# mbrea-c/bevy_firework

Measured on AMD Instinct MI355X. Metric: particles updated/sec (stress_test, 1M live), higher is better.
Workload: dtype f32; 1 GPU; configs[1]: 1 emitter x rate 1e6/s x lifetime 1 s per GPU (983 333 live), Point emission, linear 2-key scale/colour curves, dt=1/60, spawn + update + removal of the dead (order kept) every step; emitters_total=1, live_particles=983332, rccl_ranks=1, self_launched=False, update_mode=fused

## Files before the change

bevy_firework_amd/csrc/fw_engine.h:

```cpp
#pragma once
#include <hip/hip_runtime.h>

#include <algorithm>
#include <chrono>
#include <cmath>
#include <cstdio>
#include <cstdlib>
#include <cstring>
#include <string>
#include <deque>
#include <mutex>
#include <new>
#include <vector>

#include <sys/mman.h>
#include <immintrin.h>

#include "../../include/firework_hip.h"
#include "../../include/firework_hip_debug.h"
#include "fw_kernels.h"
#include "fw_math.h"
#include "fw_ages.h"
#include "fw_spin.h"
#include "fw_fuse2.h"
// ... 465 lines not shown
        if (n == cap) reserve_own(cap * 2);
        return p[n++];
    }
    void push_back(const FwOp &x) { push_slot() = x; }
    void append(const FwOp *b, const FwOp *e) {
        for (; b != e; ++b) push_back(*b);
    }
};

struct FwLevel {
    OpList g;
    std::vector<FwNestOp> n;
};

struct fw_ctx {
    std::vector<FwLevel> levels;
    OpList ops_scratch;
    std::vector<uint32_t> grow_scratch;
    HipBuf<char> d_stage;
    HipBuf<uint32_t> d_sort;
    bool seg_kind_changed = false;
    bool derive_ready_any = false;
    struct EmUndo {
        uint32_t spawner, entry;
        float last_emission, time_passed_in_cycle;
        bool enabled;
        uint64_t serial;
    };
    struct SpUndo {
        uint32_t spawner;
        uint64_t manual_queued_count;
    };
    std::vector<EmUndo> undo_em;
    std::vector<SpUndo> undo_sp;
    int device = 0;
    uint32_t seed = 0;
    HipStream stream, copy_stream;
    HipStream fifo_stream;
    HipEvent ev_side, ev_main;
    bool use_fifo_stream = true;
    bool side_dirty = false;
    bool fifo_last_side = false;
    bool main_reads_ring = false;
    std::string err;
    int update_mode = FW_MODE_FUSED;
    uint32_t spin_limit = 1u << 16;
    uint32_t dbg = 0;
    uint64_t recovered_rings = 0;

    std::vector<SpawnerHost, HugeAlloc<SpawnerHost>> spawners;
    std::vector<SegHost, HugeAlloc<SegHost>> segs;
    uint32_t n_types = 0, n_emits = 0, n_emit_slots = 0;
    std::vector<uint32_t> free_types, free_emits, free_emit_slots;
    size_t keys_end = 0;
    std::vector<std::pair<uint32_t, uint32_t>> free_keys;

    FwGlobals g{};
    struct {
        HipBuf<uint32_t> count, spawned, appended, rold;
        HipBuf<uint32_t> ndestroyed, range_ticket;
        HipBuf<uint32_t> tile_cnt, tile_off, err;
        HipBuf<unsigned long long> tile_status, dbg_ts, nest_status, nest_ticket, stats;
        HipBuf<float> tile_box;
    } gm;
    HipBuf<FwSeg> d_segs;
    HipBuf<FwType> d_types;
    HipBuf<FwTypeColl> d_type_coll;
    HipBuf<float> d_keys;
    HipBuf<FwEmit> d_emits;
    HipBuf<unsigned long long> d_emit_serial;
    HipBuf<uint32_t> d_nest_start;
    std::vector<uint32_t> nest_ticket_base;
    uint32_t max_seg = 0;
    size_t tiles_cap = 0;

    size_t param_bytes = 0;
    HipBuf<char> h_param[kParamRing];
    HipBuf<char> d_param[kParamRing];
    HipEvent ev_copied[kParamRing];
    Fence consumed[kParamRing];
    HipBuf<unsigned long long> h_done;
    unsigned long long *h_err = nullptr;
    std::string poison_msg;
    uint32_t n_poisoned = 0;
    uint64_t slot_frame[kParamRing] = {};

    HipBuf<unsigned long long> h_snap;
    bool snap_pending[kSnapRing] = {};
    bool snap_seen[kSnapRing] = {};
    uint32_t snap_epoch[kSnapRing] = {};
    std::vector<uint64_t> snap_cum[kSnapRing];

    HipBuf<uint32_t> d_tile_first;
    size_t tile_first_cap = 0;
    std::vector<uint32_t> tiles_dev;
    uint32_t total_tiles_dev = 0;
    HipBuf<uint32_t> h_tab[kTabRing];
    HipBuf<uint2> d_tile_keys;
    HipBuf<uint2> h_keys[kTabRing];
    HipBuf<uint4> d_tile_desc;
    HipBuf<uint4> h_desc[kTabRing];
    size_t tile_desc_cap = 0;
    Fence tab_fence[kTabRing];
    uint64_t tab_seq = 0, ring_seq = 0;
    uint32_t vt_rounds = 1;
    bool tab_force = false;

    uint32_t fc_sums_prev = 0;
    HipBuf<uint4> d_fce;
    HipBuf<unsigned long long> d_fc;
    size_t fc_len = 0;
    uint64_t fc_seq = 0;
    bool fc_dirty = false;
    bool fc_ok = false;
    uint32_t fc_dt_bits = 0;
    uint64_t fc_tab_seq = 0;
    bool use_forecast = true;
    bool use_tf = true;
    uint32_t tf_min_tiles = 768;
    HipBuf<uint4> d_fct;
    HipBuf<float2> d_fcl;
    size_t tf_cap = 0;
    uint32_t tf_armed = 0;
    float tf_prev_theta = 0.0f;
    uint64_t tf_frames = 0;
    bool use_static_new = true;
    bool use_stream = true;
    bool track_aabb = false;
    uint32_t boxes_epoch = 0;
    bool colors_dirty = false;
    bool use_fifo = true;
    bool fifo_nested = true;
    bool use_nospin = true;
    bool use_ageless = true;
    struct CohortTable {
        Staging<char, 1> h;
        HipBuf<char> d;
        uint64_t launches = 0;
    };
    CohortTable age_tab;
    bool use_spin_defer = true;
    uint32_t spin_defer_min = 384u * FW_TILE, spin_defer_after = 32u, spin_log_cap = 256u;
    CohortTable spin_tab;
    bool use_spinless = true;
    uint64_t spinless_launches = 0;
    bool use_whole_tiles = true;
    uint64_t whole_launches = 0, whole_tiles = 0;
    bool newborn_spin = false;
    uint64_t newborn_launches = 0;
    bool use_fuse2 = true;
    uint32_t fuse2_min = 384u * FW_TILE;
    uint32_t fuse_depth = FW_FUSE_MAX, fuse_deep_min = 768u * FW_TILE, fuse_wide_min = 768u * FW_TILE;
    uint32_t fuse_far_depth = FW_FUSE_FAR_DEFAULT, fuse_far_min = 768u * FW_TILE;
    FwWithheld withheld;
    uint64_t fused_launches = 0, fuse2_flushed = 0, fuse_frames = 0;
    bool use_axis = true;
    bool use_derived = true;
    bool derive_all = true;
    uint32_t fifo_small_tiles = 384;
    uint32_t fifo_min = 32768;
    FwPathCensus census;
    bool use_small = true;
    uint32_t small_max = 768;
    uint32_t wave_all_min = 896;
    bool wave_all_on = false;
    uint32_t wide_min = 768;
    bool wide_on = false;
    bool wide_mid_on = false;
    uint32_t wide_mid = 1400;
    uint32_t wide_max = 2048;
    uint32_t n_narrow = 0;
    uint32_t small_min = 352;
    bool small_last_side = false;
    bool small_on = false;
    bool host_fast = true;
    std::vector<uint32_t> big_list;
    bool big_dirty = true;
    std::vector<uint32_t> small_list;
    bool small_dirty = true;
    HipBuf<uint32_t> d_small, h_small;
    size_t small_cap = 0;
    Fence small_fence;
    std::vector<FwOp> fifo_ops;
    std::vector<std::pair<uint32_t, FwOp>> range_mat_ops;
    std::vector<std::pair<uint32_t, FwOp>> fifo_mat_ops;
    uint64_t tev_frames = 0;
    bool use_range = true;
    uint32_t range_min = 8192;
    uint32_t range_few = 192;
    uint32_t range_small_tiles = 384;
    bool range_small = false;
    uint32_t range_young_rounds = 4;
    uint32_t range_young_big = 0;
    std::vector<FwOp> range_ops;
    struct BirthAge {
        uint64_t frame;
        float age;
    };
    std::deque<BirthAge> birth_age;
    float range_life_max = 0.f;
    float range_age_keep = 0.f;
    HipBuf<FwRangeDesc> d_rdesc;
    HipBuf<FwRangeDesc> h_rdesc;
    size_t rdesc_cap = 0;
    uint32_t r_total = 0;
    bool r_force = true;
    Fence rtab_fence;
    HipBuf<unsigned long long> d_rstatus;
    HipBuf<char> h_rparam[kParamRing];
    bool param_bar = false;
    HipBuf<char> b_param[kParamRing];
    bool range_spread_new = true;
    uint64_t nt_bytes = 768ull << 20;
    uint64_t nt_wo_bytes = 280ull << 20, nt_wo_bytes_range = 64ull << 20;
    HipBuf<unsigned long long> d_rts;
    std::vector<uint32_t> range_scratch;
    size_t rparam_bytes = 0;
    uint64_t rslot_frame[kParamRing] = {};
    uint64_t rring_seq = 0;
    uint64_t r_uploads = 0;

    uint32_t nest_seq = 0;
    bool nest_fuse = true;
    uint64_t fused_nest_frames = 0, nest_pass_frames = 0;
    bool trace = false;
    bool host_prof = false;
    uint64_t host_prof_skip = 0;
    double prof_ns[10] = {};
    uint64_t prof_frames = 0;
    uint64_t frame = 0;
    double sim_time = 0.0;
    uint32_t parity = 0;
    unsigned long long stats_before_last = 0;
    bool stats_valid = false;

    bool timing = false;
    std::vector<HipEvent> tev;
    size_t tev_used = 0;
    uint64_t timing_particles_start = 0;
    double tev_overhead_ms = 0;

    unsigned long long *live_ring = nullptr;
    uint32_t live_ring_n = 0;
    uint64_t live_ring_frames = 0;

    HipBuf<FwCollider> d_colliders;
    uint32_t n_colliders = 0;
    Staging<FwCollider, 2> h_coll;
    struct MeshHost {
        bool alive = false;
        HipBuf<float4> nodes, tris;
        uint32_t n_nodes = 0, n_tris = 0;
        float center[3] = {0.0f, 0.0f, 0.0f}, radius = 0.0f;
        bool deformable = false;
        uint32_t n_vertices = 0;
        HipBuf<FwSlotIdx> slots;
        HipBuf<uint32_t> order, level_off;
        HipBuf<float> xyz;
        Staging<float, 2> h_xyz;
        std::vector<uint32_t> h_level_off;
        std::vector<uint8_t> referenced;
        float lo[3] = {0.0f, 0.0f, 0.0f}, hi[3] = {0.0f, 0.0f, 0.0f}, pad = 0.0f;
        HipBuf<FwMeshRecord> d_rec;
        HipBuf<FwVtxAcc> d_partials;
        HipBuf<uint8_t> d_referenced;
        HipBuf<FwMeshReport> h_report;
        bool dev_bounds = false;
        uint64_t sphere_stamp = 0;
    };
    static constexpr int kMeshDeviceAllocs = 4;
    std::vector<MeshHost> meshes;
    std::vector<fw_mesh> mesh_set;
    std::vector<fw_mesh_collider> mesh_insts;
    HipBuf<FwMeshInst> d_mesh_inst;
    Staging<FwMeshInst, 2> h_mesh_inst;
    HipBuf<float4> q_in_h, q_out_h, q_in_d, q_out_d;
    HipBuf<float4> q_out2_h, q_out2_d;
    HipBuf<float> d_aabb;
    HipBuf<float> h_aabb;
    struct {
        Staging<char, 2> h_tab;
        HipBuf<char> d_tab;
        HipBuf<float> d_part;
        HipBuf<float> h_out;
        std::vector<uint32_t> place_first;
        uint64_t launches = 0, last_chunks = 0;
    } boxes;
    struct {
        HipBuf<uint32_t> d_part;
        HipBuf<uint32_t> h_out;
        uint64_t launches = 0, last_chunks = 0;
    } volumes;
    HipBuf<unsigned long long> d_total;
    HipBuf<uint32_t> d_segids;

    uint64_t fail_alloc = 0, n_alloc = 0;

    fw_ctx() = default;
    fw_ctx(const fw_ctx &) = delete;
    fw_ctx &operator=(const fw_ctx &) = delete;
    ~fw_ctx();
};

namespace fwh {


// ... 255 lines not shown
```

bevy_firework_amd/csrc/fw_engine_api.cpp:

```cpp
#include "fw_engine.h"

thread_local std::string fwh::g_create_error;

static bool host_maps_writable(const void *p) {
    FILE *f = fopen("/proc/self/maps", "r");
    if (!f) return false;
    char line[512];
    bool ok = false;
    const unsigned long long a = (unsigned long long)(uintptr_t)p;
    while (fgets(line, sizeof line, f)) {
        unsigned long long lo = 0, hi = 0;
        char perms[8] = {0};
        if (sscanf(line, "%llx-%llx %7s", &lo, &hi, perms) == 3 && a >= lo && a < hi) {
            ok = perms[0] == 'r' && perms[1] == 'w';
            break;
        }
    }
    fclose(f);
    return ok;
}

static fw_status create_resources(fw_ctx *ctx, hipStream_t stream) {
    if (stream)
        ctx->stream.borrow(stream);
// ... 15 lines not shown
    return ensure_max_seg(ctx, 1024);
}

fw_ctx::~fw_ctx() {
    for (hipStream_t s : {(hipStream_t)stream, (hipStream_t)copy_stream, (hipStream_t)fifo_stream})
        if (s) (void)hipStreamSynchronize(s);
}

enum class Then { nothing, sync, join, counts };
enum class Ages { leave, ages, write };
struct SpawnerCall {
    SpawnerHost *sp = nullptr;
    std::vector<uint32_t> c;
    fw_status st = FW_OK;
};
template <typename ArgsOk>
static bool begin_call(fw_ctx *ctx, fw_spawner h, SpawnerCall &r, Then then, Ages ages, ArgsOk args_ok) {
    r.sp = get_spawner(ctx, h);
    if (!r.sp || !args_ok(*r.sp)) return r.st = FW_EINVAL, false;
    if (poll_device_error(ctx), r.sp->poisoned) return r.st = poisoned_status(ctx), false;
    hipSetDevice(ctx->device);
    if ((r.st = flush_withheld(ctx))) return false;
    for (size_t t = 0; ages != Ages::leave && t < r.sp->seg.size(); t++)
        if ((ages == Ages::write && (r.st = ensure_spin(ctx, r.sp->seg[t]))) || (r.st = ensure_ages(ctx, r.sp->seg[t]))) return false;
    r.st = then == Then::sync ? sync(ctx) : then == Then::join ? join_side(ctx) : then == Then::counts ? read_counts(ctx, r.c) : FW_OK;
    return !r.st || (then == Then::counts && r.st == FW_ECAPACITY);
}

static fw_status clear_poison_report(fw_ctx *ctx) {
    poll_device_error(ctx);
    ctx->h_err[0] = ctx->h_err[1] = 0ull;
    const uint32_t zero = 0;
    FW_HIP(ctx, hipMemcpy(ctx->g.err, &zero, sizeof zero, hipMemcpyHostToDevice));
    return FW_OK;
}

static void recount_poisoned(fw_ctx *ctx) {
    ctx->n_poisoned = 0;
    for (const SpawnerHost &x : ctx->spawners) ctx->n_poisoned += (x.alive && x.poisoned) ? 1u : 0u;
}

static fw_status check_handles(fw_ctx *ctx, uint32_t n, const fw_spawner *handles, const char *msg) {
    for (uint32_t i = 0; i < n; i++)
        if (!get_spawner(ctx, handles[i])) return fail(ctx, FW_EINVAL, msg);
    return FW_OK;
}

static int lplane_of(const SegHost &S, uint32_t emission_index) {
    int plane = -1;
    for (uint32_t k = 0; k < S.n_lplanes; k++)
        if (S.lplane_emission[k] == (int32_t)emission_index) plane = (int)k;
    return plane;
}

static fw_status read_stat_total(fw_ctx *ctx, uint64_t *total) {
    unsigned long long slots[FW_STAT_SLOTS];
    FW_HIP(ctx, hipMemcpy(slots, ctx->g.stats, sizeof slots, hipMemcpyDeviceToHost));
    *total = 0;
    for (unsigned long long v : slots) *total += v;
    return FW_OK;
}

extern "C" {


int fw_abi_version(void) { return FW_ABI_VERSION; }

const char *fw_last_error(const fw_ctx *ctx) { return ctx ? ctx->err.c_str() : g_create_error.c_str(); }

uint64_t fw_compute_emission_count(float t, float last, float dur, float start, float end, float per_cycle,
                                   float *next_last) {
    float nl = 0.f;
    const uint64_t n = fw_emission_count(t, last, dur, start, end, per_cycle, &nl);
    if (next_last) *next_last = nl;
    return n;
}

fw_status fw_ctx_create(int device, uint32_t seed, void *stream, fw_ctx **out) {
    if (!out) return FW_EINVAL;
    *out = nullptr;
    int ndev = 0;
    hipError_t e = hipGetDeviceCount(&ndev);
    if (e != hipSuccess || ndev <= 0) {
        g_create_error = std::string("no HIP device available (") + hipGetErrorString(e) +
                         "); this backend has no CPU fallback";
        return FW_ENODEV;
    }
    if (device < 0 || device >= ndev) {
        g_create_error = "device index out of range";
        return FW_EINVAL;
    }
    if ((e = hipSetDevice(device)) != hipSuccess) {
        g_create_error = std::string("hipSetDevice: ") + hipGetErrorString(e);
        return FW_ENODEV;
    }
    hipDeviceProp_t prop;
    if (hipGetDeviceProperties(&prop, device) == hipSuccess && strncmp(prop.gcnArchName, "gfx950", 6) != 0) {
        g_create_error = std::string("kernels are built for gfx950 only; device is ") + prop.gcnArchName;
        return FW_ENODEV;
    }
    fw_ctx *ctx = new fw_ctx();
    ctx->device = device;
    ctx->seed = seed;
    const char *knobs_on = getenv("FW_ENABLE_KNOBS");
    auto getenv = [&](const char *name) -> const char * { return (knobs_on && atoi(knobs_on) != 0) ? ::getenv(name) : nullptr; };
#ifdef FW_AB
    if (const char *m = getenv("FW_FAIL_ALLOC")) ctx->fail_alloc = strtoull(m, nullptr, 10);
#endif
    {
        int large_bar = 0;
        HipBuf<char> probe;
        if (hipDeviceGetAttribute(&large_bar, hipDeviceAttributeIsLargeBar, device) == hipSuccess && large_bar != 0 &&
            alloc_buf(ctx, probe, 4096, Mem::fine) == FW_OK) {
            hipPointerAttribute_t at{};
            ctx->param_bar = hipPointerGetAttributes(&at, probe) == hipSuccess && at.type == hipMemoryTypeDevice && host_maps_writable(probe);
        }
        (void)hipGetLastError();
        ctx->err.clear();
    }
    ctx->g.seed = seed;
    if (const char *m = getenv("FW_UPDATE_MODE")) ctx->update_mode = !strcmp(m, "split") ? FW_MODE_SPLIT : FW_MODE_FUSED;
    if (const char *m = getenv("FW_FORECAST")) ctx->use_forecast = atoi(m) != 0;
    if (const char *m = getenv("FW_TF")) ctx->use_tf = atoi(m) != 0;
    if (const char *m = getenv("FW_TF_MIN_TILES")) ctx->tf_min_tiles = (uint32_t)strtoul(m, nullptr, 10);
    if (const char *m = getenv("FW_STREAM")) ctx->use_stream = atoi(m) != 0;
    if (const char *m = getenv("FW_STATIC_NEW")) ctx->use_static_new = atoi(m) != 0;
    if (const char *m = getenv("FW_SPIN_LIMIT")) ctx->spin_limit = (uint32_t)strtoul(m, nullptr, 10);
    if (const char *m = getenv("FW_FIFO")) ctx->use_fifo = atoi(m) != 0;
    if (const char *m = getenv("FW_FIFO_MIN")) ctx->fifo_min = (uint32_t)strtoul(m, nullptr, 10);
    if (const char *m = getenv("FW_FIFO_SMALL")) ctx->fifo_small_tiles = (uint32_t)strtoul(m, nullptr, 10);
    if (const char *m = getenv("FW_FIFO_STREAM")) ctx->use_fifo_stream = atoi(m) != 0;
    if (const char *m = getenv("FW_RANGE")) ctx->use_range = atoi(m) != 0;
    if (const char *m = getenv("FW_RANGE_MIN")) ctx->range_min = (uint32_t)strtoul(m, nullptr, 10);
    if (const char *m = getenv("FW_RANGE_FEW")) ctx->range_few = (uint32_t)strtoul(m, nullptr, 10);
    if (const char *m = getenv("FW_RANGE_SMALL")) ctx->range_small_tiles = (uint32_t)strtoul(m, nullptr, 10);
    if (const char *m = getenv("FW_RANGE_YOUNG_BIG")) ctx->range_young_big = (uint32_t)strtoul(m, nullptr, 10);
    if (const char *m = getenv("FW_NOSPIN")) ctx->use_nospin = atoi(m) != 0;
    if (const char *m = getenv("FW_AXIS_SPIN")) ctx->use_axis = atoi(m) != 0;
    if (const char *m = getenv("FW_AGELESS")) ctx->use_ageless = atoi(m) != 0;
    if (const char *m = getenv("FW_SPIN_DEFER")) ctx->use_spin_defer = atoi(m) != 0;
    if (const char *m = getenv("FW_SPIN_DEFER_MIN")) ctx->spin_defer_min = (uint32_t)strtoul(m, nullptr, 10);
    if (const char *m = getenv("FW_SPIN_DEFER_AFTER")) ctx->spin_defer_after = (uint32_t)strtoul(m, nullptr, 10);
    if (const char *m = getenv("FW_SPIN_LOG")) ctx->spin_log_cap = (uint32_t)strtoul(m, nullptr, 10);
    if (const char *m = getenv("FW_SPINLESS")) ctx->use_spinless = atoi(m) != 0;
    if (const char *m = getenv("FW_WHOLE_TILES")) ctx->use_whole_tiles = atoi(m) != 0;
    if (const char *m = getenv("FW_NEWBORN_SPIN")) ctx->newborn_spin = atoi(m) != 0;
    if (const char *m = getenv("FW_FUSE2")) ctx->use_fuse2 = atoi(m) != 0;
    if (const char *m = getenv("FW_FUSE2_MIN")) ctx->fuse2_min = (uint32_t)strtoul(m, nullptr, 10);
    if (const char *m = getenv("FW_FUSE_DEPTH")) ctx->fuse_depth = (uint32_t)std::min(std::max(atoi(m), 2), (int)FW_FUSE_MAX);
    if (const char *m = getenv("FW_FUSE_DEEP_MIN")) ctx->fuse_deep_min = (uint32_t)strtoul(m, nullptr, 10);
    if (const char *m = getenv("FW_FUSE_WIDE_MIN")) ctx->fuse_wide_min = (uint32_t)strtoul(m, nullptr, 10);
    if (const char *m = getenv("FW_FUSE_FAR_DEPTH")) ctx->fuse_far_depth = (uint32_t)std::min(std::max(atoi(m), (int)FW_FUSE_MAX), (int)FW_FUSE_FAR);
    if (const char *m = getenv("FW_FUSE_FAR_MIN")) ctx->fuse_far_min = (uint32_t)strtoul(m, nullptr, 10);
    if (const char *m = getenv("FW_DERIVED")) ctx->use_derived = atoi(m) != 0, ctx->derive_all = atoi(m) >= 2;
    if (const char *m = getenv("FW_NEST_FUSE")) ctx->nest_fuse = atoi(m) != 0;
    if (const char *m = getenv("FW_SMALL")) ctx->use_small = atoi(m) != 0;
    if (const char *m = getenv("FW_SMALL_MAX")) ctx->small_max = (uint32_t)strtoul(m, nullptr, 10);
    if (const char *m = getenv("FW_SMALL_MIN")) ctx->small_min = (uint32_t)strtoul(m, nullptr, 10);
    if (const char *m = getenv("FW_WIDE_MAX")) ctx->wide_max = (uint32_t)strtoul(m, nullptr, 10);
    if (const char *m = getenv("FW_WIDE_MIN")) ctx->wide_min = (uint32_t)strtoul(m, nullptr, 10);
    if (const char *m = getenv("FW_WIDE_MID")) ctx->wide_mid = (uint32_t)strtoul(m, nullptr, 10);
    if (const char *m = getenv("FW_WAVE_ALL_MIN")) ctx->wave_all_min = (uint32_t)strtoul(m, nullptr, 10);
    if (const char *m = getenv("FW_HOST_FAST")) ctx->host_fast = atoi(m) != 0;
    if (const char *m = getenv("FW_PARAM_BAR")) ctx->param_bar = ctx->param_bar && atoi(m) != 0;
    if (const char *m = getenv("FW_NT_MB")) ctx->nt_bytes = (uint64_t)atoll(m) << 20;
    if (const char *m = getenv("FW_NT_WO_MB")) ctx->nt_wo_bytes = ctx->nt_wo_bytes_range = (uint64_t)atoll(m) << 20;
#ifdef FW_AB
    if (const char *m = getenv("FW_DEBUG")) ctx->dbg = (uint32_t)atoi(m);
    if (const char *m = getenv("FW_FIFO_NESTED")) ctx->fifo_nested = atoi(m) != 0;
    if (const char *m = getenv("FW_RANGE_SPREAD_NEW")) ctx->range_spread_new = atoi(m) != 0;
    if (const char *m = getenv("FW_AABB")) ctx->track_aabb = atoi(m) != 0;
    ctx->trace = getenv("FW_TRACE") != nullptr;
    if (const char *m = getenv("FW_HOST_PROF")) ctx->host_prof = atoi(m) != 0, ctx->host_prof_skip = atoi(m) > 1 ? (uint64_t)atoi(m) : 0;
#endif
    if (create_resources(ctx, (hipStream_t)stream) != FW_OK) {
        g_create_error = ctx->err;
        delete ctx;
        return FW_EHIP;
    }
    *out = ctx;
    return FW_OK;
}

fw_status fw_ctx_destroy(fw_ctx *ctx) {
    if (!ctx) return FW_EINVAL;
    hipSetDevice(ctx->device);
    drop_withheld(ctx);
    if (ctx->host_prof && ctx->prof_frames) {
        static const char *names[10] = {"windows+reset", "spawner loop", "tile table", "commit", "args", "op tables", "launch", "post", "", ""};
        fprintf(stderr, "[fw] host half of fw_step over %llu frames (ns per frame):", (unsigned long long)ctx->prof_frames);
        for (int i = 0; i < 8; i++) fprintf(stderr, "  %s %.0f", names[i], ctx->prof_ns[i] / (double)ctx->prof_frames);
        fprintf(stderr, "\n[fw] table uploads: general %llu, range %llu over %llu frames\n", (unsigned long long)ctx->tab_seq,
                (unsigned long long)ctx->r_uploads, (unsigned long long)ctx->frame);
        fprintf(stderr, "[fw] host records: SegHost %zu B, SpawnerHost %zu B (entry at %zu), EmissionHost %zu B, FwOp %zu B\n", sizeof(SegHost),
                sizeof(SpawnerHost), (size_t)((const char *)&ctx->spawners.data()->em.one_ - (const char *)ctx->spawners.data()),
                sizeof(EmissionHost), sizeof(FwOp));
    }
    delete ctx;
    return FW_OK;
}

void *fw_ctx_stream(const fw_ctx *ctx) { return ctx ? (void *)ctx->stream : nullptr; }

fw_status fw_ctx_synchronize(fw_ctx *ctx) {
    if (!ctx) return FW_EINVAL;
    fw_status st = sync(ctx);
    if (st) return st;
    return check_device_errors(ctx);
}

static bool collider_kind_ok(const fw_collider &c) { return c.kind >= FW_COLLIDER_PLANE && c.kind <= FW_COLLIDER_CAPSULE; }
static FwCollider collider_record(const fw_collider &c) {
    FwCollider d{};
    d.kind = c.kind, d.layers = c.layers, d.radius = c.radius;
    d.bound = c.kind == FW_COLLIDER_SPHERE ? c.radius
              : c.kind == FW_COLLIDER_BOX ? std::sqrt(c.half_extents[0] * c.half_extents[0] + c.half_extents[1] * c.half_extents[1] + c.half_extents[2] * c.half_extents[2]) * 1.0001f
              : (c.kind == FW_COLLIDER_CYLINDER || c.kind == FW_COLLIDER_CONE) ? std::sqrt(c.radius * c.radius + c.half_extents[1] * c.half_extents[1]) * 1.0001f
              : c.kind == FW_COLLIDER_CAPSULE ? (c.half_extents[1] + c.radius) * 1.0001f
                            : INFINITY;
    if (!(d.bound >= 0.0f)) d.bound = INFINITY;
    memcpy(d.position, c.position, sizeof c.position);
    memcpy(d.rotation, c.rotation, sizeof c.rotation);
    memcpy(d.normal, c.normal, sizeof c.normal);
    memcpy(d.half_extents, c.half_extents, sizeof c.half_extents);
    return d;
}

fw_status fw_ctx_set_colliders(fw_ctx *ctx, const fw_collider *colliders, uint32_t n) {
    if (!ctx || (n && !colliders)) return fail(ctx, FW_EINVAL, "bad collider set");
    hipSetDevice(ctx->device);
    if (fw_status fst = flush_withheld(ctx)) return fst;
    for (uint32_t i = 0; i < n; i++)
        if (!collider_kind_ok(colliders[i])) return fail(ctx, FW_EINVAL, "unknown collider kind");
    const size_t ncap = std::max<size_t>(64, (size_t)n * 2);
    FwCollider *h;
    fw_status st = ctx->h_coll.take(ctx, n, ncap, &h);
    if (st) return st;
    if (n > ctx->d_colliders.cap()) {
        if ((st = sync(ctx)) || (st = alloc_buf(ctx, ctx->d_colliders, ncap, Mem::device, false, &ctx->g.colliders))) return st;
    }
    for (uint32_t i = 0; i < n; i++) h[i] = collider_record(colliders[i]);
    if (n) {
        FW_HIP(ctx, hipMemcpyAsync(ctx->d_colliders, h, n * sizeof(FwCollider), hipMemcpyHostToDevice, ctx->stream));
        if ((st = ctx->h_coll.commit(ctx, ctx->stream))) return st;
    }
    ctx->n_colliders = n;
    ctx->g.n_colliders = n;
    drop_forecast_and_boxes(ctx);
    return FW_OK;
}

fw_status fw_spawner_create(fw_ctx *ctx, const fw_spawner_desc *desc, fw_spawner *out) {
    if (!ctx || !out) return FW_EINVAL;
    hipSetDevice(ctx->device);
    if (fw_status fst = flush_withheld(ctx)) return fst;
    fw_status st = validate_desc(ctx, desc);
    if (st) return st;
    if ((st = sync(ctx))) return st;
    int h = -1;
    for (size_t i = 0; i < ctx->spawners.size(); i++)
        if (!ctx->spawners[i].alive) {
            h = (int)i;
            break;
        }
    if (h < 0) {
        ctx->spawners.push_back(SpawnerHost{});
        h = (int)ctx->spawners.size() - 1;
    }
    ctx->spawners[h] = SpawnerHost{};
    ctx->spawners[h].alive = true;
    st = build_spawner(ctx, h, desc, nullptr);
    if (st) {
        release_spawner_segments(ctx, ctx->spawners[h]);
        ctx->spawners[h].alive = false;
        return st;
    }
    *out = h;
    return FW_OK;
}

fw_status fw_spawner_update_settings(fw_ctx *ctx, fw_spawner h, const fw_spawner_desc *desc) {
    SpawnerHost *sp = get_spawner(ctx, h);
    if (!sp) return FW_EINVAL;
    hipSetDevice(ctx->device);
    if (fw_status fst = flush_withheld(ctx)) return fst;
    fw_status st = validate_desc(ctx, desc);
    if (st) return st;
    if ((st = sync(ctx))) return st;
    if (sp->poisoned && (st = clear_poison_report(ctx))) return st;
    std::vector<uint64_t> serials;
    for (const EmissionHost &e : sp->em) {
        unsigned long long s = e.serial;
        if (e.es.mode == FW_MODE_NESTED)
            hipMemcpy(&s, ctx->d_emit_serial + e.emit_slot, sizeof s, hipMemcpyDeviceToHost);
        serials.push_back(s);
    }
    if ((st = release_spawner_segments(ctx, *sp))) return st;
    const bool finished_notified = sp->finished_notified;
    SpawnerHost keep = *sp;
    *sp = SpawnerHost{};
    sp->alive = true;
    sp->manual_queued_count = keep.manual_queued_count;
    memcpy(sp->origin_pos, keep.origin_pos, sizeof keep.origin_pos);
    memcpy(sp->origin_rot, keep.origin_rot, sizeof keep.origin_rot);
    memcpy(sp->parent_vel, keep.parent_vel, sizeof keep.parent_vel);
    sp->mod_scale = keep.mod_scale, sp->mod_speed = keep.mod_speed;
// ... 905 lines not shown
```

bevy_firework_amd/csrc/fw_engine_launch.cpp:

```cpp
#include "fw_engine.h"

namespace fwh {

fw_status ensure_ring(fw_ctx *ctx, FwFrame &fr, size_t bytes) {
    if (bytes > ctx->param_bytes && fr.pre_slot >= 0) {
        ctx->levels[0].g.reserve_own(ctx->levels[0].g.size());
        fr.pre_slot = -1, fr.pre_hdr = nullptr, fr.pre_hdr_ok = false;
    }
    return ensure_param_ring(ctx, bytes);
}

}

namespace {

uint32_t next_nest_seq(fw_ctx *ctx) {
    ctx->nest_seq = (ctx->nest_seq + 1u) & 0x3FFFFFFFu;
    if (!ctx->nest_seq) ctx->nest_seq = 1u;
    return ctx->nest_seq;
}

void sort_by_segment(FwOp *b, FwOp *e) {
    if (!std::is_sorted(b, e, [](const FwOp &x, const FwOp &y) { return x.seg < y.seg; }))
        std::stable_sort(b, e, [](const FwOp &x, const FwOp &y) { return x.seg < y.seg; });
// ... 220 lines not shown
                op.ticket_base = ctx->nest_ticket_base[op.emit_slot], ctx->nest_ticket_base[op.emit_slot] += op.n_tiles;
                h_nops[ni++] = op;
            }
            launches.push_back(Launch{true, first, ni - first, tiles});
        }
    }
    flush_global();
    bool staged = false;
    for (const Launch &L : launches) staged |= L.count > FW_INLINE_OPS;
    if (staged) {
        FW_HIP(ctx, hipMemcpyAsync(dp, hp, bytes, hipMemcpyHostToDevice, ctx->copy_stream));
        FW_HIP(ctx, hipEventRecord(ctx->ev_copied[fr.slot], ctx->copy_stream));
        FW_HIP(ctx, hipStreamWaitEvent(ctx->stream, ctx->ev_copied[fr.slot], 0));
    }
    for (const Launch &L : launches) {
        const bool inl_ops = L.count <= FW_INLINE_OPS;
        if (!L.nested) {
            FW_HIP(ctx, fw_launch_spawn(ctx->stream, ctx->g, inl_ops ? nullptr : (const FwOp *)dp + L.first,
                                        h_ops + L.first, (uint32_t)L.count, L.blocks, p));
        } else {
            const uint32_t tag = next_nest_seq(ctx);
            FW_HIP(ctx, fw_launch_nested(ctx->stream, ctx->g,
                                         inl_ops ? nullptr : (const FwNestOp *)(dp + off_nops) + L.first,
                                         h_nops + L.first, (uint32_t)L.count, L.blocks, p, tag,
                                         ctx->spin_limit, ctx->dbg));
        }
    }
    if (!staged) fr.slot = -1;
    if (!n_virtual) return FW_OK;
    const size_t off_ops = (size_t)n_seg * sizeof(OpHdr);
    bool others = false;
    for (size_t li = 1; li < levels.size(); li++)
        for (const FwOp &op : levels[li].g) others |= stays_virtual(op);
    OpList &g0 = levels[0].g;
    int tslot = -1;
    char *tp = nullptr;
    if (fr.pre_slot >= 0 && g0.lent && !others && fr.pre_hdr_ok && fr.pre_tracked == g0.size()) {
        tslot = fr.pre_slot, tp = ctx->h_param[tslot];
    } else {
        OpList &ops = ctx->ops_scratch;
        ops.clear();
        ops.reserve_own(n_virtual);
        for (auto &L : levels)
            for (const FwOp &op : L.g)
                if (stays_virtual(op)) ops.push_back(op);
        sort_by_segment(ops.begin(), ops.end());
        const size_t tbytes = off_ops + ops.size() * sizeof(FwOp);
        if ((st = ensure_ring(ctx, fr, tbytes))) return st;
        if ((st = acquire_slot(ctx, &tslot))) return st;
        const bool bar = ctx->param_bar && tbytes <= kBarParamBytes;
        tp = bar ? ctx->b_param[tslot] : ctx->h_param[tslot];
        write_op_headers((OpHdr *)tp, n_seg, ops.data(), ops.size());
        memcpy(tp + off_ops, ops.data(), ops.size() * sizeof(FwOp));
        if (bar) drain_bar_writes(tp);
    }
    fr.small_hdr = (const uint4 *)tp, fr.small_ops = (const FwOp *)(tp + off_ops);
    fr.small_tslot = tslot;
    return FW_OK;
}

fw_status op_table(fw_ctx *ctx, FwFrame &fr) {
    auto &levels = ctx->levels;
    FwUpdateArgs &a = fr.a;
    const uint32_t n_seg = fr.n_seg;
    fw_status st = FW_OK;
    OpList *one = nullptr;
    size_t n_lists = 0;
    for (auto &L : levels)
        if (!L.g.empty()) one = &L.g, n_lists++;
    if (n_lists != 1) {
        one = &ctx->ops_scratch;
        one->clear();
        one->reserve_own(fr.n_g);
        for (auto &L : levels) one->append(L.g.begin(), L.g.end());
    }
    OpList &ops = *one;
    const bool in_place = fr.pre_slot >= 0 && one == &levels[0].g && ops.lent;
    const bool hdr_done = in_place && fr.pre_hdr_ok && fr.pre_tracked == ops.size();
    if (!hdr_done) sort_by_segment(ops.begin(), ops.end());
    a.n_ops = (uint32_t)ops.size();
    if (ops.size() <= FW_INLINE_OPS && (ops.empty() || !ctx->census.n_small)) {
        fr.spawn_form = ops.empty() ? FW_SPAWN_NONE : FW_SPAWN_INLINE;
        for (size_t i = 0; i < ops.size(); i++) fr.inl.ops[i] = ops[i];
        return FW_OK;
    }
    fr.spawn_form = FW_SPAWN_TABLE;
    const size_t off_ops = (size_t)n_seg * sizeof(OpHdr);
    const size_t bytes = off_ops + ops.size() * sizeof(FwOp);
    int slot = fr.pre_slot;
    if (!in_place) {
        if ((st = ensure_ring(ctx, fr, bytes))) return st;
        if ((st = acquire_slot(ctx, &slot))) return st;
    }
    const bool bar = !in_place && ctx->param_bar && bytes <= kBarParamBytes;
    char *hp = bar ? ctx->b_param[slot] : ctx->h_param[slot];
    if (!hdr_done) write_op_headers((OpHdr *)hp, n_seg, ops.data(), ops.size());
    if (!in_place) memcpy(hp + off_ops, ops.data(), ops.size() * sizeof(FwOp));
    if (bar) drain_bar_writes(hp);
    a.seg_op_first = (const uint4 *)hp;
    a.ops = (const FwOp *)(hp + off_ops);
    ctx->slot_frame[slot] = ctx->frame + 1;
    fr.small_hdr = a.seg_op_first, fr.small_ops = a.ops;
    return FW_OK;
}

template <class Cohort>
fw_status take_report(fw_ctx *ctx, uint32_t si, Cohort &c, const char *what) {
    const SegHost &S = ctx->segs[si];
    if (!wait_report(S, c.frame)) FW_HIP(ctx, hipStreamSynchronize(ctx->stream));
    if (!report_landed(S, c.frame)) return poison_segment(ctx, si, what);
    c.n = (uint32_t)*(const volatile unsigned long long *)(S.h_report + (c.frame % kReportRing)), c.known = true;
    return FW_OK;
}

void group_launched(fw_ctx *ctx, const FwFifoLaunch &L) {
    const uint32_t n_withheld = L.depth - 1u;
    for (uint32_t j = 0; j < L.fa.n_segs; j++) {
        if (L.fa.s[j].seg >= ctx->segs.size()) continue;
        SegHost &S = ctx->segs[L.fa.s[j].seg];
        for (auto c = S.coh.rbegin(); ctx->newborn_spin && n_withheld && c != S.coh.rend() && c->frame >= L.frame[0]; ++c)
            for (uint32_t f = 0; f < n_withheld; f++)
                if (c->frame == L.frame[f]) c->spin_from = L.spin_from[j];
        S.fuse_last = L.depth >= 2u ? L.depth : 0u;
    }
}

void count_whole_tiles(fw_ctx *ctx, const FwFifoArgs &fa) {
    if (!fa.fuse_pad[FW_FIFO_WHOLE] || fa.dbg != 0u) return;
    uint64_t n = 0;
    for (uint32_t j = 0; j < fa.n_segs; j++) {
        const FwFifoSeg &F = fa.s[j];
        if (F.mat) continue;
        if (fa.fused >= 2u && !(F.type_idx & FW_TYPE_IDX_AGELESS)) continue;
        const uint32_t live_tiles = F.n_tiles - std::min(F.n_tiles, F.n_vt_a + F.n_vt_b);
        n += fw_fifo_whole_span(F.capacity, FW_TILE, F.head, F.n_in, F.dead, F.tile0, live_tiles).count;
    }
    ctx->whole_tiles += n, ctx->whole_launches += n ? 1u : 0u;
}
void count_newborn(fw_ctx *ctx, const FwFifoArgs &fa) {
    bool any = false;
    for (uint32_t j = 0; j < fa.n_segs; j++) {
        const FwFifoSeg &F = fa.s[j];
        any |= fa.q0pl != 0u && fa.fuse_pad[FW_FIFO_NEWBORN] != 0u && (F.type_idx & FW_TYPE_IDX_NOSPIN) != 0u && (F.type_idx & FW_TYPE_IDX_AXIS) != 0u && F.mat == 0u;
    }
    ctx->newborn_launches += any ? 1u : 0u;
}

fw_status enqueue_fifo(fw_ctx *ctx, const FwFifoLaunch &L, hipStream_t stream, hipEvent_t e0, hipEvent_t e1) {
    const bool fused = L.depth >= 2u;
    group_launched(ctx, L);
    if (fused) ctx->fused_launches++, ctx->fuse_frames += L.depth;
    else if (L.held) ctx->fuse2_flushed++;
    count_whole_tiles(ctx, L.fa), count_newborn(ctx, L.fa);
    if (L.depth > FW_FUSE_MAX)
        FW_HIP(ctx, fw_launch_update_fifo_far(stream, ctx->g, L.fa, L.fio, L.fz, L.far, L.tiles, L.nt, e0, e1));
    else
        FW_HIP(ctx, fw_launch_update_fifo(stream, ctx->g, L.fa, L.fio, L.tiles, L.nt, e0, e1, fused ? &L.fz : nullptr));
    return FW_OK;
}

}

namespace fwh {

fw_status flush_withheld(fw_ctx *ctx) {
    const FwFifoLaunch *L = ctx->withheld.take();
    return L ? enqueue_fifo(ctx, *L, ctx->stream, nullptr, nullptr) : FW_OK;
}

void drop_withheld(fw_ctx *ctx) { ctx->withheld.drop(); }

}

namespace {


struct FifoFrame {
    hipStream_t stream;
    bool small, coll_real;
    bool coll;
};

struct FifoAccum {
    FwFifoLaunch L;
    uint64_t bytes = 0;
    bool nospin = true;
    bool derived = true;
    bool fusable = true;
    bool deep = true;
    bool wide = true;
    bool far = true;
    uint32_t n_launches = 0;
    bool sent = false;

    void restart() {
        const uint32_t n = n_launches;
        *this = FifoAccum{};
        n_launches = n;
    }
    struct Words {
        bool candidate;
        uint32_t depth_max;
    };
    Words derive(const fw_ctx *ctx, bool quiet) {
        FwFifoArgs &fa = L.fa;
        fa.spinless = (ctx->use_spinless && nospin && fa.q0pl && !fa.any_inst && !fa.small_tiles) ? 1u : 0u;
        fa.fuse_pad[FW_FIFO_WHOLE] = (ctx->use_whole_tiles && fa.spinless && derived && fa.write_mask == 0) ? 1u : 0u;
        fa.fuse_pad[FW_FIFO_NEWBORN] = ctx->newborn_spin ? 0u : 1u;        L.nt = bytes > ctx->nt_bytes ? 2 : bytes > ctx->nt_wo_bytes ? 1 : 0;
        const bool candidate = fw_fuse2_candidate(ctx->use_fuse2, quiet, n_launches == 0 && fa.n_segs == ctx->census.n_fifo, fa.spinless != 0u, fusable);
        const uint32_t depth_knob = std::max(2u, std::min(ctx->fuse_depth, (uint32_t)FW_FUSE_MAX));
        const bool go_far = deep && wide && far && ctx->fuse_depth == (uint32_t)FW_FUSE_MAX && fa.fuse_pad[FW_FIFO_NEWBORN] != 0u && ctx->fuse_far_depth > (uint32_t)FW_FUSE_MAX;
        if (go_far) return Words{candidate, std::min(ctx->fuse_far_depth, (uint32_t)FW_FUSE_FAR)};
        return Words{candidate, !deep ? 2u : !wide ? std::min(depth_knob, (uint32_t)FW_FUSE_NARROW) : depth_knob};
    }
};

struct RingInput {
    bool mat_frame;
    bool mat;
    uint32_t n_spawn;
    uint32_t n_in;
};
RingInput ring_input(const SegHost &S, const FwFrame &fr) {
    RingInput in;
    in.mat_frame = S.fifo_mat && fr.nested_frame && !S.virt_parent;
    in.mat = S.fifo_dev || in.mat_frame;
    in.n_spawn = in.mat_frame ? 0u : S.frame_spawn;
    in.n_in = S.fifo_dev ? 0xFFFFFFFFu : S.ub - in.n_spawn;
    return in;
}

struct NestRole {
    int parent = -1, child = -1;
    bool any() const { return parent >= 0 || child >= 0; }
};
NestRole nest_role(const FwFrame &fr, uint32_t si) {
    NestRole r;
    for (uint32_t k = 0; fr.fuse && k < fr.n_fuse; k++) {
        if (fr.fuse_plan[k].parent_seg == si) r.parent = (int)k;
        if (fr.fuse_plan[k].child_seg == si) r.child = (int)k;
    }
    return r;
}

struct RingRules {
    bool ageless, spin_defer, newborn_defer;
    uint64_t spin_from_new;
};
fw_status ring_rules(fw_ctx *ctx, uint32_t si, float dt, const FifoFrame &ff, const RingInput &in, bool nest_touches, RingRules &R) {
    SegHost &S = ctx->segs[si];
    fw_status st = FW_OK;
    R.ageless = ctx->use_ageless && S.q0pl && ctx->fifo_small_tiles != 0u && !ff.small && !ff.coll_real && S.inst == nullptr && !S.collides && !S.fifo_dev && !S.fifo_mat &&
                !S.nested_fed && S.n_lplanes == 0 && !nest_touches && S.derived && S.destroyed == nullptr && ageless_dt_ok(dt);
    if (!R.ageless && (st = ensure_ages(ctx, si, ff.stream))) return st;
    if (R.ageless) S.ages_stale = true;
    S.ageless_last = R.ageless;
    const bool spin_ok = R.ageless && ctx->use_spin_defer && S.axis != 0u && axis_dt_ok(S, dt) && spin_dt_ok(dt) && in.n_in >= ctx->spin_defer_min &&
                         !(S.frame_spawn && !S.coh.empty() && S.coh.back().age == 0.0f);
    R.spin_defer = spin_ok && S.spin_streak >= ctx->spin_defer_after;
    if (!spin_ok) {
        if ((st = ensure_spin(ctx, si, ff.stream))) return st;
    } else if (!R.spin_defer) {
        S.spin_streak++;
    } else if (fw_spin_full(S.spin.log.size(), std::max(1u, ctx->spin_log_cap)) && (st = ensure_spin(ctx, si, ff.stream, true))) {
        return st;
    }
    R.newborn_defer = fw_spin_newborn_deferred(R.spin_defer, !in.mat, ctx->newborn_spin);
    R.spin_from_new = R.spin_defer ? S.spin.defer_spawn(S.coh, dt, R.newborn_defer) : S.spin.end();
    S.spin_last = R.spin_defer;
    return FW_OK;
}

fw_status age_cohorts(fw_ctx *ctx, uint32_t si, float dt, uint64_t spin_from_new, uint32_t *dead) {
    SegHost &S = ctx->segs[si];
    fw_status st = FW_OK;
    if (S.fifo_dev) {
        S.coh.push_back(SegHost::Cohort{0u, 0.0f, ctx->frame, false});
    } else if (S.frame_spawn) {
        if (!S.coh.empty() && S.coh.back().age == 0.0f && !std::signbit(S.coh.back().age))
            S.coh.back().n += S.frame_spawn;
        else
            S.coh.push_back(SegHost::Cohort{S.frame_spawn, 0.0f, ctx->frame, true, spin_from_new});
    }
    for (auto &c : S.coh) c.age = c.age + dt;
    *dead = 0;
    while (!S.coh.empty() && S.coh.front().age >= S.fifo_life) {
        SegHost::Cohort &c = S.coh.front();
        if (!c.known && c.frame != ctx->frame && (st = take_report(ctx, si, c, "cohort report missing"))) return st;
        *dead += c.n;
        S.coh.pop_front();
    }
    if (S.spin.stale) S.spin.trim(S.coh);
    return FW_OK;
}

void ring_record(fw_ctx *ctx, const FifoFrame &ff, FifoAccum &acc, uint32_t si, float dt, const RingInput &in, const RingRules &R, uint32_t dead,
                 bool nest_parent) {
    SegHost &S = ctx->segs[si];
    FwFifoArgs &fa = acc.L.fa;
    const int32_t wm = S.derived ? 0 : S.fifo_wm;
    if (!fa.n_segs) fa.write_mask = wm;
    else if (fa.write_mask != wm) fa.write_mask = -1;
    acc.fusable &= R.spin_defer && in.n_in >= ctx->fuse2_min && (R.newborn_defer || ctx->newborn_spin);
    acc.deep &= in.n_in >= ctx->fuse_deep_min;
    acc.wide &= in.n_in >= ctx->fuse_wide_min;
    acc.far &= in.n_in >= ctx->fuse_far_min;
    acc.L.spin_from[fa.n_segs] = R.spin_from_new;
    memcpy(acc.L.fz.move[fa.n_segs], S.fifo_move, sizeof S.fifo_move);
    FwFifoSeg &F = fa.s[fa.n_segs++];
    F.buf = S.buf[0], F.destroyed = S.destroyed, F.inst = S.inst;
    F.inst_cap = S.inst_cap, F.capacity = S.capacity, F.seg = si;
    if (S.axis != 0u && !axis_dt_ok(S, dt)) S.axis = 0u;
    F.type_idx = S.type_idx | ((S.nospin || R.spin_defer) ? FW_TYPE_IDX_NOSPIN : 0u) | (S.axis << FW_TYPE_IDX_AXIS_SHIFT) | (R.ageless ? FW_TYPE_IDX_AGELESS : 0u), F.life = S.fifo_life;
    F.keys_off = S.keys_off, F.keys_len = S.keys_len;
    F.head = S.head, F.n_in = in.n_in, F.n_spawn = in.n_spawn, F.dead = dead;
    F.mat = in.mat ? 1u : 0u;
    fa.q0pl = S.q0pl ? 1u : 0u;
    acc.nospin &= (F.type_idx & FW_TYPE_IDX_NOSPIN) != 0u;
    acc.derived &= S.derived;
    F.n_lplanes = S.n_lplanes;
    F.report = S.fifo_dev ? S.h_report + (ctx->frame % kReportRing) : nullptr;
    F.op0 = acc.L.n_ops;
    if (!in.mat_frame)
        for (const FwOp &op : ctx->fifo_ops)
            if (op.seg == si) acc.L.fio.ops[acc.L.n_ops++] = op;
    F.op1 = acc.L.n_ops;
    const uint32_t n_old = S.fifo_dev ? S.capacity : in.n_in;
    const uint32_t lo = std::min((S.destroyed || nest_parent) ? 0u : dead, n_old);
    const uint32_t ftile = ff.coll ? FW_FIFO_COLL_TILE : FW_TILE;
    const FwFifoLayout L = fw_fifo_layout(S.capacity, ftile, FW_BLOCK, S.head, lo, n_old, S.fifo_dev ? 0u : in.n_in, in.n_spawn);
    F.spawn_a = L.spawn_a, F.n_vt_a = L.n_vt_a, F.n_vt_b = L.n_vt_b, F.tile0 = L.tile0, F.n_tiles = L.n_tiles;
    F.tile_first = acc.L.tiles;
    acc.L.tiles += F.n_tiles;
    F.nest = 0u;
    acc.bytes += (uint64_t)L.live_tiles * ftile * (S.nospin ? 104u : 164u);
    fa.any_inst |= S.inst != nullptr ? 1u : 0u;
    fa.any_coll |= (ff.coll_real && !S.q0pl) ? 1u : 0u;
    fa.small_tiles = (ff.coll && !(ff.coll_real && !S.q0pl)) ? 1u : 0u;
    S.head = (uint32_t)(((uint64_t)S.head + dead) % S.capacity);
    if (!S.fifo_dev) S.ub = in.n_in + in.n_spawn - std::min(dead, in.n_in + in.n_spawn);
}

void wire_nest(fw_ctx *ctx, const FwFrame &fr, FwFifoArgs &fa, const NestRole &nest, uint32_t nest_tag, uint32_t *status_next) {
    FwFifoSeg &F = fa.s[fa.n_segs - 1u];
    if (nest.parent >= 0) {
        const FwNestOp &op = fr.fuse_plan[nest.parent];
        FwFifoNest &N = fa.nest[nest.parent];
        F.nest = (uint32_t)nest.parent + 1u;
        N.parent = fa.n_segs - 1u;
        N.emit = op.emit, N.emit_slot = op.emit_slot, N.parent_lplane = op.parent_lplane;
        N.n_count = op.n_count, N.n_start = op.n_start, N.n_end = op.n_end, N.speed = op.speed, N.scale = op.scale;
        N.status_first = *status_next, N.n_ptiles = F.n_tiles - (F.n_vt_a + F.n_vt_b);
        *status_next += N.n_ptiles;
        N.ticket_base = ctx->nest_ticket_base[op.emit_slot], ctx->nest_ticket_base[op.emit_slot] += N.n_ptiles;
        N.tag = nest_tag, N.spin_limit = ctx->spin_limit;
        fa.n_nest = fr.n_fuse;
    }
    if (nest.child >= 0) {
        F.nest = ((uint32_t)nest.child + 1u) | FW_FIFO_NEST_CHILD;
        fa.nest[nest.child].child = fa.n_segs - 1u;
    }
}

fw_status launch_fifo(fw_ctx *ctx, FwFrame &fr) {
    const FwUpdateArgs &a = fr.a;
    const float dt = fr.dt;
    const uint32_t n_seg = fr.n_seg;
    bool side = ctx->use_fifo_stream && ctx->stream.owned() && (fr.total_tiles != 0 || ctx->census.n_small != 0) && ctx->live_ring == nullptr;
    for (const SegHost &S : ctx->segs) side &= !(S.in_use && S.fifo && (S.fifo_mat || S.inst != nullptr || S.collides));
    fw_status st = order_side(ctx, side, ctx->fifo_last_side);
    if (st) return st;
    const bool quiet = fr.quiet && fr.spawn_form == FW_SPAWN_NONE && !side;
    if (!quiet && (st = flush_withheld(ctx))) return st;
    FifoFrame ff;
    ff.stream = side ? ctx->fifo_stream : ctx->stream;
    ff.small = !fr.ring_stats.fifo_dev && fr.ring_stats.fifo_parts < (uint64_t)ctx->fifo_small_tiles * FW_TILE;
    ff.coll_real = fr.ring_stats.fifo_coll;
    ff.coll = ff.coll_real || ff.small;
    FifoAccum acc{};
    FwFifoArgs &fa = acc.L.fa;
    uint32_t nest_status_next = 0;
    const uint32_t nest_tag = fr.fuse ? next_nest_seq(ctx) : 0u;
    auto flush = [&]() -> fw_status {
        if (acc.sent || !fa.n_segs) return FW_OK;
        fa.parity = fr.p, fa.epoch = a.epoch, fa.dbg = ctx->dbg, fa.dt = dt;
        fa.done_tag = side ? nullptr : a.done_tag, fa.done_value = a.done_value;
        fa.host_counts = a.host_counts;
        fa.live_out = a.live_out, fa.live_next = a.live_next;
        const FifoAccum::Words w = acc.derive(ctx, quiet);
        acc.n_launches++;
        fr.fifo_launched = true;
        fw_status fst = FW_OK;
        const FwOffered o = ctx->withheld.offer(acc.L, w.candidate, w.depth_max, ctx->frame);
        if (o.first && (fst = enqueue_fifo(ctx, *o.first, ff.stream, nullptr, nullptr))) {
            ctx->withheld.drop();
            return fst;
        }
        ctx->spinless_launches += fa.spinless;
        if (o.withheld) fr.snap = -1, fr.a.host_counts = nullptr;
        if (o.second) {
            hipEvent_t e0 = nullptr, e1 = nullptr;
            if (o.second->depth == 1u) next_timing_pair(ctx, fr, &e0, &e1);
            if ((fst = enqueue_fifo(ctx, *o.second, ff.stream, e0, e1))) return fst;
        }
        if (side) ctx->side_dirty = true;
        acc.sent = true;
        return FW_OK;
    };
    for (int pass = 0; pass < 2; pass++) {
        for (uint32_t si = 0; si < n_seg; si++) {
            const SegHost &S = ctx->segs[si];
            if (!S.in_use || !S.fifo || S.q0pl != (pass == 1)) continue;
            uint32_t k_ops = 0;
            for (const FwOp &op : ctx->fifo_ops) k_ops += op.seg == si ? 1u : 0u;
            if (k_ops > FW_INLINE_OPS)
                return poison_segment(ctx, si, "a FIFO ring with more spawn ops than its launch can carry");
            if ((fa.n_segs == FW_FIFO_PER_LAUNCH || acc.L.n_ops + k_ops > FW_INLINE_OPS) && (st = flush())) return st;
            if (acc.sent) acc.restart();
            const RingInput in = ring_input(S, fr);
            const NestRole nest = nest_role(fr, si);
            RingRules rules;
            uint32_t dead = 0;
            if ((st = ring_rules(ctx, si, dt, ff, in, nest.any(), rules))) return st;
            if ((st = age_cohorts(ctx, si, dt, rules.spin_from_new, &dead))) return st;
            ring_record(ctx, ff, acc, si, dt, in, rules, dead, nest.parent >= 0);
            wire_nest(ctx, fr, fa, nest, nest_tag, &nest_status_next);
        }
        if ((st = flush())) return st;
    }
    return FW_OK;
}

inline bool fit(uint32_t &have, uint32_t need, uint32_t spare, uint32_t &low) {
    if (need > have) {
        have = need + spare, low = 0;
        return true;
    }
    if (have > need + need / 4 + spare + 2) {
        if (++low > 64) {
            have = need + spare, low = 0;
            return true;
        }
    } else {
        low = 0;
    }
    return false;
}

fw_status launch_range(fw_ctx *ctx, FwFrame &fr) {
    const FwUpdateArgs &a = fr.a;
    const float dt = fr.dt;
    const uint32_t n_seg = fr.n_seg;
    const int rslot = (int)(ctx->rring_seq++ % kParamRing);
    fw_status st = wait_slot_free(ctx, ctx->rslot_frame[rslot]);
    if (st) return st;
    FwRangeRec *recs = (FwRangeRec *)ctx->h_rparam[rslot].get();
    FwOp *rops = (FwOp *)(ctx->h_rparam[rslot] + round_up((uint32_t)(ctx->max_seg * sizeof(FwRangeRec)), 64));
    std::vector<FwOp> &ops = ctx->range_ops;
    sort_by_segment(ops.data(), ops.data() + ops.size());
    if (!ops.empty()) memcpy(rops, ops.data(), ops.size() * sizeof(FwOp));
    bool dirty = ctx->r_force, all_nospin = true, range_inst = false, range_coll = false;
    {
        const uint64_t parts = fr.ring_stats.range_parts;
        const bool any_dev = fr.ring_stats.range_dev, any_coll_r = fr.ring_stats.range_coll;
        const uint64_t lim = (uint64_t)ctx->range_small_tiles * FW_TILE;
        const bool small = any_coll_r || (!any_dev && parts < (ctx->range_small ? lim + lim / 4 : lim));
        if (small != ctx->range_small) ctx->range_small = small, dirty = true;
        const uint64_t mean = parts / std::max<uint32_t>(1u, ctx->census.n_range), big = ctx->range_young_big;
        uint32_t yr = ctx->range_young_rounds;
        if (small || any_dev || fr.ring_stats.range_inst || big == 0) yr = 4;
        else if (yr == 4 && mean >= big) yr = 2;
        else if (yr == 2 && mean < big - big / 4) yr = 4;
        if (yr != ctx->range_young_rounds) ctx->range_young_rounds = yr, dirty = true;
    }
    const uint32_t OT = ctx->range_small ? (uint32_t)FW_BLOCK : (uint32_t)FW_TILE;
    uint64_t r_bytes = 0;
    size_t oi = 0;
    for (uint32_t si = 0; si < n_seg; si++) {
        SegHost &S = ctx->segs[si];
        if (!S.in_use || !S.range) continue;
        all_nospin &= S.nospin;
        range_inst |= S.inst != nullptr;
        range_coll |= S.collides;
        r_bytes += (uint64_t)(S.range_dev ? S.capacity / 2 : S.ub) * (S.nospin ? 104u : 164u);
        S.dead_at_end = true;
        const bool mat_frame = S.range_mat && fr.nested_frame && !S.virt_parent;
        uint32_t grad = 0;
        if (!S.range_dev) {
            while (!S.ycoh.empty()) {
                const float an = birth_age_before(ctx, S.ycoh.front().frame) + dt;
                if (an < S.range_life_lo) break;
                grad += S.ycoh.front().n;
                S.ycoh.pop_front();
            }
            if (S.frame_spawn) S.ycoh.push_back(SegHost::YCohort{ctx->frame, S.frame_spawn});
        } else {
            while (!S.dcoh.empty()) {
                SegHost::DCohort &c = S.dcoh.front();
                const float an = birth_age_before(ctx, c.frame) + dt;
                if (an < S.range_life_lo) break;
                if (!c.known && (st = take_report(ctx, si, c, "cohort report missing (range ring)"))) return st;
                grad += c.n;
                if (c.n) S.gcoh.push_back(SegHost::YCohort{c.frame, c.n}), S.gcoh_sum += c.n;
                S.dcoh.pop_front();
            }
            S.dcoh.push_back(SegHost::DCohort{ctx->frame, 0u, false});
            while (!S.gcoh.empty() && !(birth_age_before(ctx, S.gcoh.front().frame) < (float)S.life_bound)) {
                S.gcoh_sum -= S.gcoh.front().n;
                S.gcoh.pop_front();
            }
        }
        {
            uint64_t nb = (uint64_t)S.young_lo + grad;
            while (nb >= S.capacity) nb -= S.capacity;
            S.young_lo = (uint32_t)nb;
        }
        const uint32_t y_exist = S.range_dev ? 0u : S.young_n - std::min(S.young_n, grad);
        FwRangeRec Rc{};
        Rc.b = S.young_lo, Rc.y_exist = y_exist, Rc.n_spawn = (mat_frame || S.range_dev) ? 0u : S.frame_spawn;
        Rc.grad = grad, Rc.flags = (mat_frame ? FW_RREC_MAT : 0u) | (S.range_dev ? (FW_RREC_MAT | FW_RREC_DEV) : 0u);
        Rc.report = S.range_dev ? S.h_report + (ctx->frame % kReportRing) : nullptr, Rc.pad2 = 0;
        while (oi < ops.size() && ops[oi].seg < si) oi++;
        Rc.op0 = (uint32_t)oi, Rc.op_n = 0;
        while (oi < ops.size() && ops[oi].seg == si) oi++, Rc.op_n++;
        S.young_n = S.range_dev ? 0u : y_exist + S.frame_spawn;
        const uint32_t YT = ctx->range_small ? (uint32_t)FW_BLOCK : ctx->range_young_rounds * (uint32_t)FW_BLOCK;
        const uint32_t ysh = (uint32_t)__builtin_ctz(YT), osh = (uint32_t)__builtin_ctz(OT);
        uint32_t need_old, need_new, need_young;
        if (S.range_dev) {
            need_old = std::max<uint32_t>(1u, (uint32_t)std::min<uint64_t>((S.gcoh_sum + OT - 1) >> osh, (S.capacity >> osh) + 1));
            need_new = 0u;
            need_young = S.capacity >> ysh;
// ... 167 lines not shown
```

bevy_firework_amd/csrc/fw_engine_step.cpp:

```cpp
#include "fw_engine.h"

namespace {


fw_status begin_frame(fw_ctx *ctx, float dt) {
    poll_device_error(ctx);
    if (ctx->n_poisoned)
        for (const SpawnerHost &sp : ctx->spawners)
            if (sp.alive && sp.poisoned) return poisoned_status(ctx);
    poll_snapshots(ctx);
    if (ctx->derive_ready_any) {
        ctx->derive_ready_any = false;
        for (uint32_t i = 0; i < ctx->segs.size(); i++) {
            SegHost &S = ctx->segs[i];
            if (!S.in_use || !S.derive_ready) continue;
            S.derive_ready = false;
            if (S.colors_dirty || !wants_derived(ctx, S)) continue;
            const fw_status dst = set_derived(ctx, i, true);
            if (dst) return dst;
        }
    }

    for (auto &L : ctx->levels) L.g.clear(), L.n.clear();
    ctx->fifo_ops.clear(), ctx->fifo_mat_ops.clear(), ctx->range_mat_ops.clear();
// ... 281 lines not shown
                        else pre_hdr_ok = false;
                        pre_tracked = idx + 1u;
                    }
                    fill(G.push_slot());
                } else {
                    FwOp op;
                    fill(op);
                    if (S.fifo && S.fifo_mat && !S.virt_parent)
                        ctx->fifo_mat_ops.push_back({(uint32_t)i, op});
                    else if (S.fifo)
                        ctx->fifo_ops.push_back(op);
                    else if (S.range_mat && !S.virt_parent)
                        ctx->range_mat_ops.push_back({(uint32_t)i, op});
                    else
                        ctx->range_ops.push_back(op);
                }
                E.serial += n;
                if (!S.solo) S.frame_spawn += (uint32_t)n;
                S.ub = (uint32_t)std::min<uint64_t>((uint64_t)S.ub + n, 0xFFFFFFFFull);
                if (S.small && S.ub > ctx->small_max && !S.wide) {
                    S.wide = true, S.wide_big = false, ctx->small_dirty = true;
                    if (!ctx->wide_mid_on) {
                        const bool was_solo = S.solo;
                        small_deactivate(ctx, S);
                        if (was_solo) S.frame_spawn = (uint32_t)n;
                    }
                }
                if (S.small && S.wide && S.ub > std::max(ctx->small_max, 2u * ctx->wide_max)) {
                    const bool was_solo = S.solo;
                    leave_small(ctx, S);
                    if (was_solo) S.frame_spawn = (uint32_t)n;
                }
                note_spawned(ctx, S, n);
            } else {
                if (es.pacing_kind != FW_PACING_COUNT_OVER_DURATION) continue;
                const SegHost &P = ctx->segs[sp.seg[es.target_particle_type]];
                if (!(dt < E.life_lo_safe)) new_static = false;
                FwNestOp op{};
                op.parent_seg = sp.seg[es.target_particle_type], op.child_seg = dst;
                op.emit = E.emit_idx, op.emit_slot = E.emit_slot;
                {
                    const uint32_t par_ub = P.nested_fed ? P.capacity : std::min(P.ub, P.capacity);
                    op.n_tiles = (par_ub + FW_NEST_TILE - 1) / FW_NEST_TILE + 1;
                }
                op.speed = sp.mod_speed, op.scale = sp.mod_scale;
                for (uint32_t k = 0; k < P.n_lplanes; k++)
                    if (P.lplane_emission[k] == (int32_t)i) op.parent_lplane = k;
                op.n_count = es.count, op.n_start = es.offset_start, op.n_end = es.offset_end;
                levels[i].n.push_back(op);
            }
        }
    }
    fr.new_static = new_static, fr.pre_hdr_ok = pre_hdr_ok, fr.pre_tracked = pre_tracked;
    return FW_OK;
}

void route_ring_ops(fw_ctx *ctx, FwFrame &fr) {
    auto &levels = ctx->levels;
    for (auto &L : levels) fr.nested_frame |= !L.n.empty();
    for (auto &io : ctx->fifo_mat_ops) {
        if (fr.nested_frame) {
            io.second.head = ctx->segs[io.second.seg].enqueue_head();
            levels[io.first].g.push_back(io.second);
        } else {
            ctx->fifo_ops.push_back(io.second);
        }
    }
    for (auto &io : ctx->range_mat_ops) {
        if (fr.nested_frame) {
            io.second.head = ctx->segs[io.second.seg].enqueue_head(), io.second.range_ring = 1u;
            levels[io.first].g.push_back(io.second);
        } else {
            ctx->range_ops.push_back(io.second);
        }
    }
    ctx->fifo_mat_ops.clear(), ctx->range_mat_ops.clear();

    if (!ctx->seg_kind_changed) return;
    auto reroute = [&](std::vector<FwOp> &list, bool was_fifo) {
        size_t w = 0;
        for (size_t r = 0; r < list.size(); r++) {
            const FwOp &op = list[r];
            const SegHost &S = ctx->segs[op.seg];
            if (was_fifo ? S.fifo : S.range) {
                list[w++] = op;
                continue;
            }
            size_t lvl = 0;
            const SpawnerHost &osp = ctx->spawners[S.spawner];
            for (size_t i = 0; i < osp.em.size(); i++)
                if (osp.em[i].emit_idx == op.emit) lvl = i;
            levels[lvl].g.push_back(op);
            if (!(fr.dt < osp.em[lvl].life_lo_safe)) fr.new_static = false;
        }
        list.resize(w);
    };
    reroute(ctx->fifo_ops, true);
    reroute(ctx->range_ops, false);
    for (auto &L : levels)
        for (FwOp &op : L.g)
            if (op.range_ring && !ctx->segs[op.seg].range) op.range_ring = 0u, op.head = 0u;
}

void plan_fuse(fw_ctx *ctx, FwFrame &fr) {
    const float dt = fr.dt;
    if (fr.nested_frame && ctx->nest_fuse && !fr.any_coll && !ctx->seg_kind_changed && ctx->update_mode == FW_MODE_FUSED && ctx->census.n_fifo != 0 &&
        ctx->census.n_fifo <= FW_FIFO_PER_LAUNCH && ctx->fifo_ops.size() <= FW_INLINE_OPS && !fr.ring_stats.fifo_coll && !fr.ring_stats.fifo_inst &&
        dt >= 0.0f && std::isfinite(dt)) {
        bool fuse = true;
        for (auto &L : ctx->levels) {
            for (const FwOp &op : L.g) fuse &= !ctx->segs[op.seg].ring();
            for (const FwNestOp &op : L.n) {
                if (!fuse || fr.n_fuse == FW_FIFO_NEST_MAX) {
                    fuse = false;
                    break;
                }
                const SegHost &P = ctx->segs[op.parent_seg], &Cs = ctx->segs[op.child_seg];
                const uint32_t p_in = P.ub - std::min(P.ub, P.frame_spawn);
                fuse = P.fifo && !P.fifo_dev && P.virt_parent && P.n_lplanes == 1 && Cs.fifo && Cs.fifo_dev && Cs.n_lplanes == 0 &&
                       op.parent_seg < op.child_seg && Cs.capacity <= FW_RANGE_MAX_CAPACITY &&
                       (uint64_t)(P.head % FW_TILE) + p_in <= P.capacity;
                for (uint32_t k = 0; k < fr.n_fuse; k++)
                    fuse &= fr.fuse_plan[k].parent_seg != op.parent_seg && fr.fuse_plan[k].parent_seg != op.child_seg &&
                            fr.fuse_plan[k].child_seg != op.parent_seg && fr.fuse_plan[k].child_seg != op.child_seg;
                if (fuse) fr.fuse_plan[fr.n_fuse++] = op;
            }
            if (!fuse) break;
        }
        fr.fuse = fuse && fr.n_fuse != 0;
    }
    if (fr.nested_frame) (fr.fuse ? ctx->fused_nest_frames : ctx->nest_pass_frames)++;
}

fw_status finish_plan(fw_ctx *ctx, FwFrame &fr) {
    fr.prof(ctx, 1);
    fr.n_seg = (uint32_t)ctx->segs.size();
    fw_status st = update_tile_table(ctx);
    fr.prof(ctx, 2);
    if (st) return st;
    fr.total_tiles = ctx->total_tiles_dev;
    if (fr.total_tiles > ctx->tiles_cap) return fail(ctx, FW_EHIP, "internal error: the tile table exceeds the tile scratch (frame not enqueued)");
    for (auto &L : ctx->levels) fr.n_g += L.g.size(), fr.n_n += L.n.size();
    return ensure_ring(ctx, fr, (size_t)fr.n_seg * 16 + fr.n_g * sizeof(FwOp) + fr.n_n * sizeof(FwNestOp) + 16);
}

}

extern "C" {

fw_status fw_step(fw_ctx *ctx, float dt) {
    if (!ctx) return FW_EINVAL;
    hipSetDevice(ctx->device);
    FwFrame fr;
    fr.prof_t = std::chrono::steady_clock::now();
    fr.dt = dt;
    fw_status st = begin_frame(ctx, dt);
    if (!st) st = recover_missing_reports(ctx, dt);
    if (!st) st = segment_pass(ctx, fr);
    if (st) return st;
    ctx->undo_em.clear(), ctx->undo_sp.clear();
    if ((st = take_op_slot(ctx, fr))) return st;
    fr.prof(ctx, 0);
    st = spawner_loop(ctx, fr);
    if (!st) {
        route_ring_ops(ctx, fr);
        plan_fuse(ctx, fr);
        st = finish_plan(ctx, fr);
    }
    if (st) return rollback(ctx, st);
    fr.prof(ctx, 3);
    return enqueue_frame(ctx, fr);
}

}
```

bevy_firework_amd/csrc/fw_fuse2.h:

```cpp
#pragma once
#include <stdint.h>

#ifndef FW_HD
#ifdef __HIPCC__
#define FW_HD __host__ __device__ __forceinline__
#else
#define FW_HD inline
#endif
#endif

struct FwFifoFrame {
    uint32_t head, n_in, n_spawn, dead;
};

struct FwFifoLayout {
    uint32_t tile0, live_tiles, spawn_a, n_vt_a, n_vt_b, n_tiles;
};
FW_HD FwFifoLayout fw_fifo_layout(uint32_t capacity, uint32_t tile, uint32_t block, uint32_t head, uint32_t lo, uint32_t n_old, uint32_t first_new,
                                  uint32_t n_spawn) {
    FwFifoLayout L;
    const uint32_t cnt = n_old - lo;
    const uint32_t ps = (uint32_t)(((uint64_t)head + lo) % capacity), ring_tiles = capacity / tile;
    const uint32_t ns0 = (uint32_t)(((uint64_t)head + first_new) % capacity);
    L.spawn_a = n_spawn < capacity - ns0 ? n_spawn : capacity - ns0;
    L.n_vt_a = (L.spawn_a + block - 1) / block, L.n_vt_b = (n_spawn - L.spawn_a + block - 1) / block;
    L.tile0 = ps / tile;
    const uint32_t need = (ps % tile + cnt + tile - 1) / tile;
    L.live_tiles = cnt ? (ring_tiles < need ? ring_tiles : need) : 0u;
    L.n_tiles = L.n_vt_a + L.n_vt_b + L.live_tiles;
    if (L.n_tiles == 0u) L.n_tiles = 1u;
    return L;
}

FW_HD bool fw_fifo_tile_whole(uint32_t capacity, uint32_t tile, uint32_t head, uint32_t n_in, uint32_t dead, uint32_t pt) {
    const uint32_t s0 = pt * tile;
    if (n_in > capacity || dead > n_in) return false;
    if (head > s0 && head - s0 < tile) return dead == 0u && n_in == capacity;
    const uint32_t i0 = s0 >= head ? s0 - head : s0 + (capacity - head);
    return i0 >= dead && i0 + tile <= n_in;
}

struct FwWholeSpan {
    uint32_t count, first, len;
};
FW_HD uint32_t fw_overlap(uint32_t a0, uint32_t a1, uint32_t b0, uint32_t b1) {
    const uint32_t lo = a0 > b0 ? a0 : b0, hi = a1 < b1 ? a1 : b1;
    return hi > lo ? hi - lo : 0u;
}
FW_HD FwWholeSpan fw_fifo_whole_span(uint32_t capacity, uint32_t tile, uint32_t head, uint32_t n_in, uint32_t dead, uint32_t tile0, uint32_t live_tiles) {
    FwWholeSpan W{0u, 0u, 0u};
    const uint32_t ring_tiles = capacity / tile;
    if (n_in > capacity || dead > n_in) return W;
    if (dead == 0u && n_in == capacity) {
        W.len = ring_tiles;
    } else {
        const uint64_t lo = ((uint64_t)head + dead + tile - 1u) / tile, hi = ((uint64_t)head + n_in) / tile;
        W.first = (uint32_t)(lo % ring_tiles), W.len = hi > lo ? (uint32_t)(hi - lo) : 0u;
    }
    const uint32_t off = W.first >= tile0 ? W.first - tile0 : W.first + (ring_tiles - tile0);
    W.count = fw_overlap(off, off + W.len, 0u, live_tiles) + fw_overlap(off, off + W.len, ring_tiles, ring_tiles + live_tiles);
    return W;
}

FW_HD bool fw_fuse2_candidate(bool enabled, bool quiet, bool only_launch, bool spinless, bool unread_and_large) {
    return enabled && quiet && only_launch && spinless && unread_and_large;
}

FW_HD bool fw_fuse2_ok(uint32_t capacity, const FwFifoFrame &A, const FwFifoFrame &B) {
    if (A.head >= capacity || A.n_in > capacity || A.n_spawn > capacity - A.n_in) return false;
    if (A.dead > A.n_in) return false;
    if (B.head != (uint32_t)(((uint64_t)A.head + A.dead) % capacity) || B.n_in != A.n_in + A.n_spawn - A.dead) return false;
    if ((uint64_t)A.dead + B.dead > A.n_in) return false;
    if ((uint64_t)A.n_in + A.n_spawn + B.n_spawn > capacity) return false;
    return true;
}

FW_HD FwFifoFrame fw_fuse2_frame(const FwFifoFrame &A, const FwFifoFrame &B) { return FwFifoFrame{A.head, A.n_in, A.n_spawn + B.n_spawn, A.dead + B.dead}; }

#define FW_FUSE_MAX 8
#define FW_FUSE_NARROW 4
struct FwFuseGroup {
    FwFifoFrame U;
    uint32_t depth;
    uint32_t spawn_end[FW_FUSE_MAX];
    uint32_t dead[FW_FUSE_MAX];
};
FW_HD FwFuseGroup fw_fuse_begin(const FwFifoFrame &A) {
    FwFuseGroup G{};
    G.U = A, G.depth = 1u, G.spawn_end[0] = A.n_spawn, G.dead[0] = A.dead;
    return G;
}
FW_HD bool fw_fuse_push(uint32_t capacity, FwFuseGroup &G, const FwFifoFrame &B) {
    if (G.depth < 1u || G.depth >= FW_FUSE_MAX || !fw_fuse2_ok(capacity, G.U, B)) return false;
    G.U = fw_fuse2_frame(G.U, B);
    G.spawn_end[G.depth] = G.U.n_spawn, G.dead[G.depth] = B.dead;
    G.depth++;
    return true;
}

#define FW_FUSE_FAR 16
#define FW_FUSE_FAR_DEFAULT 16
struct FwFarGroup {
    FwFifoFrame U;
    uint32_t depth;
    uint32_t spawn_end[FW_FUSE_FAR];
    uint32_t dead[FW_FUSE_FAR];
};
FW_HD FwFarGroup fw_far_begin(const FwFifoFrame &A) {
    FwFarGroup G{};
    G.U = A, G.depth = 1u, G.spawn_end[0] = A.n_spawn, G.dead[0] = A.dead;
    return G;
}
FW_HD bool fw_far_push(uint32_t capacity, FwFarGroup &G, const FwFifoFrame &B) {
    if (G.depth < 1u || G.depth >= FW_FUSE_FAR || !fw_fuse2_ok(capacity, G.U, B)) return false;
    G.U = fw_fuse2_frame(G.U, B);
    G.spawn_end[G.depth] = G.U.n_spawn, G.dead[G.depth] = B.dead;
    G.depth++;
    return true;
}
```

bevy_firework_amd/csrc/fw_k_rings.hip:

```cpp
#include "fw_dev.h"

template <bool INST, bool NT = false>
__device__ __forceinline__ void fw_fifo_inst_out(const FwFifoSeg &F, char *inst, const float4 *s_inst_wave, const float4 *rec,
                                                 uint32_t lane, unsigned long long m, bool alive, uint32_t o) {
    if (!INST || inst == nullptr || m == 0ull) return;
    const uint32_t cnt = (uint32_t)__popcll(m);
    const uint32_t o_first = __builtin_amdgcn_readlane(o, __ffsll((long long)m) - 1);
    const uint32_t o_last = __builtin_amdgcn_readlane(o, 63 - __clzll((long long)m));
    if (o_last - o_first + 1u == cnt) {
        fw_inst_flush<NT>(inst, F.inst_cap, s_inst_wave, lane, m, o_first);
    } else {
        __builtin_amdgcn_fence(__ATOMIC_RELEASE, "wavefront");
        __builtin_amdgcn_wave_barrier();
        __builtin_amdgcn_fence(__ATOMIC_ACQUIRE, "wavefront");
        if (alive && o < F.inst_cap)
            for (uint32_t k = 0; k < 4; k++) fw_st4(inst + (size_t)o * 64u, k, rec[k]);
        __builtin_amdgcn_fence(__ATOMIC_RELEASE, "wavefront");
        __builtin_amdgcn_wave_barrier();
    }
}

struct FwCollArm {
    bool on;
    float restitution, friction;
// ... 2 lines not shown
template <int COLL>
__device__ __forceinline__ FwCollArm fw_coll_arm(const FwGlobals &g, uint32_t type_idx) {
    if constexpr (COLL) {
        const FwTypeColl TC = g.type_coll[type_idx];
        return FwCollArm{(TC.coll_flags & FW_COLL_ENABLED) != 0u, TC.coll_restitution, TC.coll_friction, TC.coll_mask};
    } else {
        return FwCollArm{false, 0.0f, 0.0f, 0u};
    }
}
template <int COLL>
__device__ __forceinline__ void fw_coll_step(const FwGlobals &g, const FwCollArm &A, bool active, float dt, float4 q0, float4 q1,
                                             fw_v3 *cpos, fw_v3 *cvel) {
    *cpos = fw_v3{q0.x, q0.y, q0.z}, *cvel = fw_v3{q1.x, q1.y, q1.z};
    if constexpr (COLL) {
        if (A.on && active) fw_particle_collision(cpos, cvel, dt, A.restitution, A.friction, false, A.mask, g.colliders, g.n_colliders, g.mesh_inst,
                                                  COLL == 2 ? g.n_mesh_inst : 0u);
    }
}

template <int R, int NT>
__device__ __forceinline__ void fw_fifo_nest_parents(const FwGlobals &g, const FwFifoArgs &a, const FwFifoNest &N, const FwFifoSeg &F,
                                                     const FwFifoSeg &Fc, uint32_t rank, uint32_t sbase, uint32_t n_in) {
    constexpr int BLK = FW_BLOCK, NW = BLK / 64, LBW = 4;
    __shared__ uint32_t s_w[R][NW];
    __shared__ uint32_t s_lb[2 * LBW * NW];
    __shared__ uint32_t s_inc[R][NW][64];
    __shared__ uint32_t s_n[R][BLK];
    __shared__ __attribute__((aligned(16))) float4 s_par[NW][3][64];
    __shared__ __attribute__((aligned(16))) float s_ckeys[FW_KEYS_MAX];
    const uint32_t tid = threadIdx.x, lane = tid & 63u, wave = tid >> 6;
    const uint32_t C = F.capacity, head = F.head, Cc = Fc.capacity;
    char *pb = F.buf;
    const char *w0 = pb + FW_OFF_Q0(C) + (size_t)sbase * 16u, *w1 = pb + FW_OFF_Q1(C) + (size_t)sbase * 4u;
    const char *w2 = pb + FW_OFF_Q2(C) + (size_t)sbase * 4u;
    char *wl = pb + FW_OFF_L(C, N.parent_lplane) + (size_t)sbase * 4u;
    const bool pnospin = (F.type_idx & FW_TYPE_IDX_NOSPIN) != 0u;
    float p_age[R], p_lea[R];
#pragma unroll
    for (int r = 0; r < R; r++) {
        const uint32_t o = (uint32_t)(r * BLK) + tid;
        p_age[r] = fw_ld1w(w0, o * 16u + 12u);
        p_lea[r] = fw_ld1w(wl, o * 4u);
    }
    const uint32_t cidx = a.parity * g.max_seg + Fc.seg;
    const uint32_t cbase = g.count[cidx] + g.spawned[cidx] + g.appended[cidx];
    const unsigned long long serial0 = g.emit_serial[N.emit_slot];
    const FwEmit &e = g.emits[N.emit];
    const FwType Tc = g.types[Fc.type_idx & FW_TYPE_IDX_MASK];
    for (uint32_t i = tid; i < Fc.keys_len; i += BLK) s_ckeys[i] = g.keys[Fc.keys_off + i];
#pragma unroll
    for (int r = 0; r < R; r++) {
        const uint32_t o = (uint32_t)(r * BLK) + tid, s = sbase + o;
        uint32_t i = s - head;
        if (s < head) i += C;
        uint32_t nr = 0;
        if (i < n_in) {
            float next;
            const uint64_t cnt = fw_emission_count(p_age[r], p_lea[r], F.life, N.n_start, N.n_end, N.n_count, &next);
            nr = cnt > 0xFFFFFFFFull ? 0xFFFFFFFFu : (uint32_t)cnt;
            fw_st1w(wl, o * 4u, next);
        }
        uint32_t x = nr;
#pragma unroll
        for (int d = 1; d < 64; d <<= 1) {
            const uint32_t u = __shfl_up(x, d, 64);
            if (lane >= (uint32_t)d) x = (x + u < x) ? 0xFFFFFFFFu : x + u;
        }
        s_n[r][tid] = nr, s_inc[r][wave][lane] = x;
        if (lane == 63) s_w[r][wave] = x;
    }
    __syncthreads();
    unsigned long long tot64 = 0;
#pragma unroll
    for (int r = 0; r < R; r++)
#pragma unroll
        for (int w = 0; w < NW; w++) tot64 += s_w[r][w];
    uint32_t tile_total = tot64 > 0xFFFFFFFFull ? 0xFFFFFFFFu : (uint32_t)tot64;
    {
        const uint32_t d0 = __builtin_amdgcn_readfirstlane(cbase), d1 = __builtin_amdgcn_readfirstlane((uint32_t)serial0),
                       d2 = __builtin_amdgcn_readfirstlane((uint32_t)(serial0 >> 32));
        asm volatile("; fw_fifo_nest_parents: counters read before the tile publishes" : "+v"(tile_total) : "s"(d0), "s"(d1), "s"(d2));
    }
    const uint32_t tile = N.status_first + rank;
    const bool lb_needed = rank != 0u;
    if (lb_needed && tid == 0) __hip_atomic_store(&g.nest_status[tile], fw_pack_status(N.tag, FW_ST_AGG, tile_total), RLX, AGENT);
    uint32_t excl = 0;
    if (lb_needed) {
        bool timed_out = false;
        excl = fw_lookback<BLK, NW, LBW>(g.nest_status, N.status_first, tile, N.tag, N.spin_limit * 64u + 1024u, s_lb, &timed_out);
        if (timed_out && tid == 0) fw_raise(g, 6u, F.seg, tile);
    }
    const unsigned long long incl64 = (unsigned long long)excl + tile_total;
    if (tid == 0)
        __hip_atomic_store(&g.nest_status[tile], fw_pack_status(N.tag, FW_ST_INCL, incl64 > 0xFFFFFFFFull ? 0xFFFFFFFFu : (uint32_t)incl64), RLX, AGENT);
    if (tile_total == 0u) return;
    const FwOutWin Wc = fw_out_window(Fc.buf, Cc, 0u, Tc, 0u, 0u, true, true);
    float4 prot = make_float4(0.0f, 0.0f, 0.0f, 1.0f);
    if (pnospin) {
        const FwType &Tp = g.types[F.type_idx & FW_TYPE_IDX_MASK];
        prot = make_float4(Tp.const_rot[0], Tp.const_rot[1], Tp.const_rot[2], Tp.const_rot[3]);
    }
    uint32_t run = excl;
#pragma unroll 1
    for (int r = 0; r < R; r++) {
        uint32_t woff = run;
#pragma unroll
        for (int w = 0; w < NW; w++) {
            if ((uint32_t)w < wave) woff += s_w[r][w];
            run += s_w[r][w];
        }
        const uint32_t tw = s_w[r][wave];
        if (tw == 0) continue;
        if (s_n[r][tid] != 0) {
            const uint32_t o16 = ((uint32_t)(r * BLK) + tid) * 16u;
            s_par[wave][0][lane] = fw_ld4w(w0, o16);
            s_par[wave][1][lane] = fw_ldc3w(w1, FW_CP(C), o16 / 4u, 0.0f);
            s_par[wave][2][lane] = pnospin ? prot : fw_ldc4w(w2, FW_CP(C), o16 / 4u);
        }
        __builtin_amdgcn_fence(__ATOMIC_RELEASE, "wavefront");
        __builtin_amdgcn_wave_barrier();
        __builtin_amdgcn_fence(__ATOMIC_ACQUIRE, "wavefront");
        for (uint32_t c0 = 0; c0 < tw; c0 += 64u) {
            const uint32_t c = c0 + lane;
            if (c < tw) {
                uint32_t lo = 0, hi = 63;
                while (lo < hi) {
                    const uint32_t mid = (lo + hi) >> 1;
                    if (s_inc[r][wave][mid] > c) hi = mid;
                    else lo = mid + 1;
                }
                const unsigned long long j = (unsigned long long)woff + c;
                const unsigned long long slotl = (unsigned long long)cbase + j;
                if (slotl < Cc) {
                    const float4 pq0 = s_par[wave][0][lo], pq1 = s_par[wave][1][lo], pq2 = s_par[wave][2][lo];
                    const FwSpawnOut so = fw_spawn_one(e, g.seed, serial0 + j, fw_v3{pq0.x, pq0.y, pq0.z}, fw_q4{pq2.x, pq2.y, pq2.z, pq2.w},
                                                       fw_v3{pq1.x, pq1.y, pq1.z}, N.speed, N.scale);
                    float age_new;
                    fw_survives(so.q0.w, a.dt, so.q3.w, &age_new);
                    fw_integrate_store<true, -1, NT, true>(Tc, s_ckeys, a.dt, so.q0, so.q1, so.q2, so.q3, age_new, Wc,
                                                     fw_ring_slot(Fc.head, (uint32_t)slotl, Cc), nullptr, nullptr, nullptr, nullptr, false, true, false);
                }
            }
        }
        __builtin_amdgcn_fence(__ATOMIC_RELEASE, "wavefront");
        __builtin_amdgcn_wave_barrier();
    }
}

#ifndef FW_FIFO_UNROLL
#define FW_FIFO_UNROLL 4
#endif
template <bool INST, int WM, int NT, int COLL, int TR, bool NEST, bool Q0PL = false, bool SPINLESS = false, int FUSE = 0, bool NBFACT = false>
__device__ __forceinline__ void fw_update_fifo_body(const FwGlobals &g, const FwFifoArgs &a, const FwInlineOps &inl, const FwFuseArgs *fz = nullptr,
                                                    const FwFarArgs *far = nullptr) {
    constexpr int BLK = FW_BLOCK;
    constexpr int NW = BLK / 64;
    constexpr int R = TR;
    constexpr uint32_t TILE = (uint32_t)(BLK * TR);
    __shared__ __attribute__((aligned(16))) float s_keys[FW_KEYS_MAX];
    __shared__ __attribute__((aligned(16))) float4 s_inst[INST ? NW * 256 : 1];
    const uint32_t tid = threadIdx.x, lane = tid & 63u, wave = tid >> 6;
    uint32_t j = 0;
    for (uint32_t i = 1; i < a.n_segs; i++)
        if (a.s[i].tile_first <= blockIdx.x) j = i;
    const FwFifoSeg &F = a.s[j];
    const uint32_t C = F.capacity, ring_tiles = C / TILE;
    const uint32_t tis = blockIdx.x - F.tile_first;
    const uint32_t n_vt = F.n_vt_a + F.n_vt_b;
    const bool spawner = tis < n_vt;
    uint32_t pt = F.tile0 + (tis - n_vt);
    if (pt >= ring_tiles) pt -= ring_tiles;
    const uint32_t head = F.head, n_dead = F.dead;
    const uint32_t sidx = a.parity * g.max_seg + F.seg;
    uint32_t c_cnt = 0, c_new = 0;
    if (F.mat) c_cnt = g.count[sidx], c_new = g.spawned[sidx] + g.appended[sidx];
    const uint32_t n_in = F.mat ? __builtin_amdgcn_readfirstlane(c_cnt + c_new) : F.n_in;
    const uint32_t full_from = F.mat ? __builtin_amdgcn_readfirstlane(c_cnt) : 0xFFFFFFFFu;
    const uint32_t n_tot = n_in + F.n_spawn;
    const uint32_t k0 = spawner ? (tis < F.n_vt_a ? tis * BLK : F.spawn_a + (tis - F.n_vt_a) * BLK) : 0u;
    uint32_t sbase = spawner ? head + n_in + k0 : pt * TILE;
    if (sbase >= C) sbase -= C;
    if (spawner && sbase >= C) sbase -= C;
    constexpr bool WT = SPINLESS && FUSE != 0;
    bool whole = false;
    if constexpr (WT)
        whole = !spawner && a.fuse_pad[FW_FIFO_WHOLE] != 0u && F.mat == 0u && a.dbg == 0u && (F.type_idx & FW_TYPE_IDX_AGELESS) != 0u &&
                fw_fifo_tile_whole(C, TILE, head, F.n_in, n_dead, pt);
    const float key0 = (!whole && tid < F.keys_len) ? g.keys[F.keys_off + tid] : 0.0f;
    char *buf = F.buf;
    float4 q0c, q1c, q2c, q3c, q0n, q1n, q2n, q3n;
    q0c = q1c = q2c = q3c = q0n = q1n = q2n = q3n = make_float4(0.f, 0.f, 0.f, 0.f);
    static_assert(!SPINLESS || (Q0PL && !INST && TR == FW_ROUNDS), "the spin-less form: streaming launches of rings with Q0 in planes");
    static_assert(FUSE == 0 || (SPINLESS && FUSE >= 2 && FUSE <= FW_FUSE_FAR), "several frames in one pass: the spin-less forms only, two to FW_FUSE_FAR");
    auto dt_w = [&](int f) -> float {
        if constexpr (FUSE > FW_FUSE_MAX)
            if (f >= FW_FAR_FIRST) return far->dt[f - FW_FAR_FIRST];
        return fz->dt_pre[f];
    };
    auto spawn_end_w = [&](uint32_t jj, int f) -> uint32_t {
        if constexpr (FUSE > FW_FUSE_MAX)
            if (f >= FW_FAR_FIRST) return far->spawn_end[jj][f - FW_FAR_FIRST];
        return fz->spawn_end[jj][f];
    };
    auto dead_w = [&](uint32_t jj, int f) -> uint32_t {
        if constexpr (FUSE > FW_FUSE_MAX)
            if (f >= FW_FAR_FIRST) return far->dead[jj][f - FW_FAR_FIRST];
        return fz->dead[jj][f];
    };
    const bool nospin = SPINLESS || (F.type_idx & FW_TYPE_IDX_NOSPIN) != 0u;
    const uint32_t axis = (F.type_idx & FW_TYPE_IDX_AXIS) >> FW_TYPE_IDX_AXIS_SHIFT;
    const bool ldx = !nospin && (axis == 0u || axis == 1u), ldy = !nospin && (axis == 0u || axis == 2u), ldz = !nospin && (axis == 0u || axis == 3u);
    const float4 q3s = make_float4(0.0f, 0.0f, 0.0f, F.life);
    const bool defer = F.mat != 0u && F.n_in == 0xFFFFFFFFu;
    const uint32_t i1 = (uint32_t)(min(1, R - 1) * BLK + (int)tid) * 16u;
    if constexpr (NEST) {
        if (!spawner && F.nest != 0u && !(F.nest & FW_FIFO_NEST_CHILD)) {
            const FwFifoNest &N = a.nest[F.nest - 1u];
            __shared__ uint32_t s_prank;
            if (FW_TICKETS) {
                if (tid == 0u) s_prank = atomicAdd(&g.nest_start[N.emit_slot], 1u) - N.ticket_base;
                __syncthreads();
            }
            const uint32_t prank = FW_TICKETS ? s_prank : tis - n_vt;
            pt = F.tile0 + prank;
            if (pt >= ring_tiles) pt -= ring_tiles;
            sbase = pt * TILE;
            fw_fifo_nest_parents<R, NT>(g, a, N, F, a.s[N.child], prank, sbase, n_in);
        }
    }
    const size_t sfirst = (size_t)sbase * 16u, cp = FW_CP(C);
    static_assert(!Q0PL || (!NEST && COLL == 0), "rings with Q0 in planes are launched by themselves");
    constexpr bool q0pl = Q0PL;
    const char *iw0 = buf + FW_OFF_Q0(C) + (q0pl ? sfirst / 4u : sfirst), *iw1 = buf + FW_OFF_Q1(C) + sfirst / 4u;
    const char *iw2 = buf + FW_OFF_Q2(C) + sfirst / 4u, *iw3 = buf + FW_OFF_Q3(C) + sfirst / 4u;
    const bool ageless = q0pl && (F.type_idx & FW_TYPE_IDX_AGELESS) != 0u;
    auto ld0 = [&](uint32_t o16) -> float4 {
        if (!q0pl) return fw_ld4w<NT == 2>(iw0, o16);
        float4 v = fw_ldc3w<NT == 2>(iw0, cp, o16 / 4u, 0.0f);
        if (!ageless) v.w = fw_ld1w<NT == 2>(iw0 + 3 * cp, o16 / 4u);
        return v;
    };
    auto ld1 = [&](uint32_t o16) -> float4 {
        if constexpr (INST) return fw_ldc4w<NT == 2>(iw1, cp, o16 / 4u);
        else return fw_ldc3w<NT == 2>(iw1, cp, o16 / 4u, 0.0f);
    };
    auto ld3 = [&](uint32_t o16) -> float4 {
        float4 v = q3s;
        if (ldx) v.x = fw_ld1w<NT == 2>(iw3, o16 / 4u);
        if (ldy) v.y = fw_ld1w<NT == 2>(iw3 + cp, o16 / 4u);
        if (ldz) v.z = fw_ld1w<NT == 2>(iw3 + 2 * cp, o16 / 4u);
        return v;
    };
    auto ld2 = [&](uint32_t o16) -> float4 {
        float4 v = make_float4(0.0f, 0.0f, 0.0f, 1.0f);
        if (ldx) v.x = fw_ld1w<NT == 2>(iw2, o16 / 4u);
        if (ldy) v.y = fw_ld1w<NT == 2>(iw2 + cp, o16 / 4u);
        if (ldz) v.z = fw_ld1w<NT == 2>(iw2 + 2 * cp, o16 / 4u);
        if (!nospin) v.w = fw_ld1w<NT == 2>(iw2 + 3 * cp, o16 / 4u);
        return v;
    };
    auto publish_fused = [&](uint32_t oidx) {
        if constexpr (FUSE != 0) {
            uint32_t nc_prev = n_in, nc = n_in, all_f = 0u, sp_done = 0u, dead_done = 0u;
            unsigned long long all_sum = 0ull;
#pragma unroll
            for (int f = 0; f < FUSE; f++) {
                const uint32_t sp_end = f < FUSE - 1 ? spawn_end_w(j, f) : F.n_spawn;
                const uint32_t dead_f = f < FUSE - 1 ? dead_w(j, f) : n_dead - dead_done;
                nc_prev = nc;
                all_f = nc_prev + (sp_end - sp_done);
                nc = all_f - min(dead_f, all_f);
                sp_done = sp_end, dead_done += dead_f, all_sum += all_f;
            }
            const uint32_t last = (FUSE & 1) ? oidx : sidx, other = (FUSE & 1) ? sidx : oidx;
            g.count[other] = nc_prev, g.count[last] = nc;
            g.spawned[oidx] = 0, g.spawned[sidx] = 0;
            g.appended[oidx] = 0, g.appended[sidx] = 0;
            g.ndestroyed[F.seg] = all_f - nc;
            if (a.host_counts) a.host_counts[F.seg] = ((unsigned long long)a.epoch << 32) | nc;
            if (a.live_out) atomicAdd(a.live_out, (unsigned long long)nc);
            if (!FW_DBG(a.dbg, 128u)) atomicAdd(g.stats + (F.seg % FW_STAT_SLOTS), all_sum);
        }
    };
    if constexpr (WT) {
        if (whole) {
            if (blockIdx.x == 0 && tid == 0) {
                if (a.live_next) *a.live_next = 0ull;
                if (a.done_tag) *a.done_tag = a.done_value;
            }
            float4 wq0[R], wq1[R];
#pragma unroll
            for (int r = 0; r < R; r++) {
                const uint32_t b4 = (uint32_t)(r * BLK + (int)tid) * 4u;
                wq0[r] = fw_ldc3w<NT == 2>(iw0, cp, b4, 0.0f);
                wq1[r] = fw_ldc3w<NT == 2>(iw1, cp, b4, 0.0f);
                __builtin_amdgcn_sched_barrier(0);
            }
            const FwMoveK K{{fz->move[j][0], fz->move[j][1], fz->move[j][2]}, fz->move[j][3]};
            char *ow0 = buf + FW_OFF_Q0(C) + sfirst / 4u, *ow1 = buf + FW_OFF_Q1(C) + sfirst / 4u;
#pragma unroll
            for (int r = 0; r < R; r++) {
                float4 q0w = wq0[r], q1w = wq1[r];
#pragma unroll
                for (int f = 0; f < FUSE - 1; f++) {
                    const FwMove mv = fw_move_step(K, dt_w(f), q0w, q1w);
                    q0w.x = mv.px, q0w.y = mv.py, q0w.z = mv.pz;
                    q1w.x = mv.vx, q1w.y = mv.vy, q1w.z = mv.vz;
                }
                const FwMove mv = fw_move_step(K, a.dt, q0w, q1w);
                const uint32_t b4 = (uint32_t)(r * BLK + (int)tid) * 4u;
                fw_stc3w<NT == 2>(ow0, cp, b4, mv.px, mv.py, mv.pz);
                fw_stc3w<NT == 2>(ow1, cp, b4, mv.vx, mv.vy, mv.vz);
                __builtin_amdgcn_sched_barrier(0);
            }
            if (tis == 0 && tid == 0) {
                if (g.count[sidx] != n_in) fw_raise(g, 5u, F.seg, n_in);
                if (F.report) *F.report = (unsigned long long)a.epoch << 32;
                publish_fused((a.parity ^ 1u) * g.max_seg + F.seg);
            }
            return;
        }
    }
    if (!spawner && !defer) {
        q0c = ld0(tid * 16u), q3c = ld3(tid * 16u);
        q1c = ld1(tid * 16u), q2c = ld2(tid * 16u);
        if constexpr (R > 1) {
            q0n = ld0(i1), q3n = ld3(i1);
            q1n = ld1(i1), q2n = ld2(i1);
        }
    }
    if (defer) {
        uint32_t i0 = sbase - head;
        if (sbase < head) i0 += C;
        if (tis != 0u && !(i0 < n_tot || (i0 + TILE > C && n_tot != 0u))) return;
        q0c = ld0(tid * 16u), q3c = ld3(tid * 16u);
        q1c = ld1(tid * 16u), q2c = ld2(tid * 16u);
        if constexpr (R > 1) {
            q0n = ld0(i1), q3n = ld3(i1);
            q1n = ld1(i1), q2n = ld2(i1);
        }
    }
    if (blockIdx.x == 0 && tid == 0) {
        if (a.live_next) *a.live_next = 0ull;
        if (a.done_tag) *a.done_tag = a.done_value;
    }
    FwType T = g.types[F.type_idx & FW_TYPE_IDX_MASK];
    if constexpr (Q0PL && !SPINLESS) {
        if (!spawner && nospin && axis != 0u) T.flags |= FW_TYPE_NOSPIN;
    }
    static_assert(!NBFACT || (SPINLESS && FUSE != 0), "the newborns' deferral as a fact of the code: the fused forms");
    bool nb_defer = NBFACT;
    if constexpr (Q0PL && FUSE == 0) nb_defer = spawner && a.fuse_pad[FW_FIFO_NEWBORN] != 0u && (F.type_idx & FW_TYPE_IDX_NOSPIN) != 0u && axis != 0u && F.mat == 0u;
    const FwCollArm CA = fw_coll_arm<COLL>(g, F.type_idx & FW_TYPE_IDX_MASK);
    bool bad = false;
    if (tid < F.keys_len) s_keys[tid] = key0;
    for (uint32_t i = tid + BLK; i < F.keys_len; i += BLK) s_keys[i] = g.keys[F.keys_off + i];
    __syncthreads();
// ... 52 lines not shown
        float4 *rec = (INST && inst != nullptr) ? s_inst_wave + fw_lane_prefix(m) * 4u : nullptr;
        fw_v3 cpos, cvel;
        fw_coll_step<COLL>(g, CA, alive, a.dt, so.q0, so.q1, &cpos, &cvel);
        if (alive) {
            fw_integrate_store<true, -1, NT, true>(T, s_keys, a.dt, so.q0, so.q1, so.q2, so.q3, age_new, W, s, rec, COLL ? &cpos : nullptr,
                                         COLL ? &cvel : nullptr, nullptr, false, true, CA.on, FW_W_REGS, !nb_defer);
            if (F.n_lplanes) fw_init_last_emitted(g, g.segs[F.seg], buf, s, new_ei, so.q3.w);
        } else if (is_new && want_destroyed)
            fw_store_destroyed(F.destroyed, buf, C, s, false, T, s_keys, so.q0, so.q1, so.q2, so.q3, age_new, i);
        fw_fifo_inst_out<INST, NT == 2>(F, inst, s_inst_wave, rec, lane, m, alive, i - n_dead);
    } else {
        FwType Ts;
        FwOutWin Ws;
        if constexpr (SPINLESS) {
            Ts = T, Ts.flags |= FW_TYPE_NOSPIN;
            Ws = W, Ws.wr2 = false, Ws.wr3 = false;
        }
        const FwType &Tt = SPINLESS ? Ts : T;
        const FwOutWin &Wt = SPINLESS ? Ws : W;
        if (want_destroyed && n_dead != 0u) {
#pragma unroll 1
            for (int r = 0; r < R; r++) {
                const uint32_t s = sbase + r * BLK + tid;
                uint32_t i = s - head;
                if (s < head) i += C;
                if (i < n_dead && i < n_in) {
                    const uint32_t b16 = (uint32_t)(r * BLK + (int)tid) * 16u;
                    const float4 q0 = q0pl ? fw_ldc4w<NT == 2>(iw0, cp, b16 / 4u) : fw_ld4w<NT == 2>(iw0, b16), q1 = fw_ldc4w<NT == 2>(iw1, cp, b16 / 4u);
                    const float4 q2 = nospin ? make_float4(0.0f, 0.0f, 0.0f, 1.0f) : fw_ldc4w<NT == 2>(iw2, cp, b16 / 4u);
                    const float4 q3 = nospin ? q3s : fw_ldc4w<NT == 2>(iw3, cp, b16 / 4u);
                    fw_store_destroyed(F.destroyed, buf, C, s, i < full_from, Tt, s_keys, q0, q1, q2, q3, q0.w + a.dt, i);
                }
            }
        }
#pragma unroll FW_FIFO_UNROLL
        for (int r = 0; r < R; r++) {
            const uint32_t s = sbase + r * BLK + tid;
            const uint32_t in_ = (uint32_t)(min(r + 2, R - 1) * BLK + (int)tid) * 16u;
            float4 q0f = q0c, q3f = q3c, q1f = q1c, q2f = q2c;
            if constexpr (R > 1) {
                q0f = ld0(in_), q3f = ld3(in_);
                q1f = ld1(in_), q2f = ld2(in_);
            }
            if (nospin) q3c = q3s;
            uint32_t i = s - head;
            if (s < head) i += C;
            if constexpr (FUSE != 0) {
#pragma unroll
                for (int f = 0; f < FUSE - 1; f++) {
                    const float dt_f = dt_w(f);
                    const FwMove mv = fw_move_step(Tt, dt_f, q0c, q1c);
                    q0c = make_float4(mv.px, mv.py, mv.pz, q0c.w + dt_f);
                    q1c.x = mv.vx, q1c.y = mv.vy, q1c.z = mv.vz;
                }
            }
            float age_new;
            const bool surv = fw_survives(q0c.w, a.dt, q3c.w, &age_new);
            const bool mine = i < n_in, dead = i < n_dead;
            bad |= !ageless && mine && surv == dead;
            const bool alive = mine && !dead;
            const unsigned long long m = INST ? __ballot(alive) : 0ull;
            float4 *rec = (INST && inst != nullptr) ? s_inst_wave + fw_lane_prefix(m) * 4u : nullptr;
            fw_v3 cpos, cvel;
            fw_coll_step<COLL>(g, CA, alive, a.dt, q0c, q1c, &cpos, &cvel);
            if (alive) {
                if FW_DBG(a.dbg, 2u) {
                    const uint32_t b16 = (s - Wt.first) * 16u;
                    if (Wt.q0pl) {
                        fw_stc3w<NT == 2>(Wt.q0, Wt.cp, b16 / 4u, q0c.x, q0c.y, q0c.z);
                        if (Wt.wr_age) fw_st1w<NT == 2>(Wt.q0 + 3 * Wt.cp, b16 / 4u, age_new);
                    } else {
                        fw_st4w<NT == 2>(Wt.q0, b16, make_float4(q0c.x, q0c.y, q0c.z, age_new));
                    }
                    fw_stc3w<NT == 2>(Wt.q1, Wt.cp, b16 / 4u, q1c.x, q1c.y, q1c.z);
                    if (WM >= 0 ? (WM & 1) != 0 : Wt.wr5) fw_st4w<NT != 0>(Wt.q5, b16, q0c);
                    if (WM >= 0 ? (WM & 2) != 0 : Wt.wr6) fw_st4w<NT != 0>(Wt.q6, b16, q1c);
                    if (WM >= 0 ? (WM & 4) != 0 : Tt.sc_kind != 0) fw_st1w<NT != 0>(Wt.s4, (s - Wt.first) * 4u, q1c.w);
                } else {
                    fw_integrate_store<true, WM, NT, true>(Tt, s_keys, a.dt, q0c, q1c, q2c, q3c, age_new, Wt, s, rec, COLL ? &cpos : nullptr,
                                                 COLL ? &cvel : nullptr, nullptr, false, i >= full_from, CA.on, INST ? FW_W_MEM : FW_W_MEM_LAZY);
                }
            }
            fw_fifo_inst_out<INST, NT == 2>(F, inst, s_inst_wave, rec, lane, m, alive, i - n_dead);
            q0c = q0n, q1c = q1n, q2c = q2n, q3c = q3n;
            q0n = q0f, q1n = q1f, q2n = q2f, q3n = q3f;
        }
    }
    if (__any(bad) && lane == 0) fw_raise(g, 4u, F.seg, blockIdx.x);
    uint32_t nest_total = 0u;
    if constexpr (NEST) {
        if (tis == 0u && (F.nest & FW_FIFO_NEST_CHILD) != 0u) {
            __shared__ uint32_t s_lbc[2 * 4 * NW];
            const FwFifoNest &N = a.nest[(F.nest & ~FW_FIFO_NEST_CHILD) - 1u];
            bool timed_out = false;
            if (N.n_ptiles)
                nest_total = fw_lookback<BLK, NW, 4>(g.nest_status, N.status_first, N.status_first + N.n_ptiles, N.tag,
                                                     N.spin_limit * 64u + 1024u, s_lbc, &timed_out);
            if (timed_out && tid == 0) fw_raise(g, 6u, F.seg, N.status_first + N.n_ptiles);
        }
    }
    if (tis == 0 && tid == 0) {
        const uint32_t oidx = (a.parity ^ 1u) * g.max_seg + F.seg;
        if (F.mat ? (F.n_in != 0xFFFFFFFFu && F.n_in != n_in) : g.count[sidx] != n_in)
            fw_raise(g, 5u, F.seg, n_in);
        uint32_t n_all = n_tot, added = c_new;
        if constexpr (NEST) {
            if ((F.nest & FW_FIFO_NEST_CHILD) != 0u) {
                const FwFifoNest &N = a.nest[(F.nest & ~FW_FIFO_NEST_CHILD) - 1u];
                const uint32_t room = C - min(C, n_tot);
                if (nest_total > room) fw_flag(g, FW_ERR_CAPACITY);
                const uint32_t take = min(nest_total, room);
                g.emit_serial[N.emit_slot] += (unsigned long long)nest_total;
                n_all += take, added += take;
            }
        }
        if (F.report) *F.report = ((unsigned long long)a.epoch << 32) | added;
        if constexpr (FUSE != 0) {
            publish_fused(oidx);
            return;
        }
        const uint32_t nc = n_all - min(n_dead, n_all);
        g.count[oidx] = nc;
        g.spawned[oidx] = 0;
        g.appended[oidx] = 0;
        g.ndestroyed[F.seg] = n_all - nc;
        if (a.host_counts) a.host_counts[F.seg] = ((unsigned long long)a.epoch << 32) | nc;
        if (a.live_out) atomicAdd(a.live_out, (unsigned long long)nc);
        if (!FW_DBG(a.dbg, 128u)) atomicAdd(g.stats + (F.seg % FW_STAT_SLOTS), (unsigned long long)n_all);
    }
}

#ifndef FW_FIFO_WAVES
#define FW_FIFO_WAVES 1
#endif
template <bool INST, int WM, int NT = 0, int COLL = 0, int TR = FW_ROUNDS, bool Q0PL = false, bool SPINLESS = false>
__global__ __launch_bounds__(FW_BLOCK) __attribute__((amdgpu_waves_per_eu((!INST && !COLL && TR == FW_ROUNDS) ? FW_FIFO_WAVES : (COLL == 1 && TR == 1) ? 4 : 1)))
void fw_k_update_fifo(FwGlobals g, FwFifoArgs a, FwInlineOps inl) {
    fw_update_fifo_body<INST, WM, NT, COLL, TR, false, Q0PL, SPINLESS>(g, a, inl);
}
template <int D, int WM, int NT>
__global__ __launch_bounds__(FW_BLOCK) __attribute__((amdgpu_waves_per_eu(FW_FIFO_WAVES))) void fw_k_update_fifo2(FwGlobals g, FwFifoArgs a, FwInlineOps inl, FwFuseArgs fz) {
    fw_update_fifo_body<false, WM, NT, 0, FW_ROUNDS, false, true, true, D, true>(g, a, inl, &fz);
}
template <int D, int WM, int NT>
__global__ __launch_bounds__(FW_BLOCK) __attribute__((amdgpu_waves_per_eu(FW_FIFO_WAVES))) void fw_k_update_fifo2_eager(FwGlobals g, FwFifoArgs a, FwInlineOps inl, FwFuseArgs fz) {
    fw_update_fifo_body<false, WM, NT, 0, FW_ROUNDS, false, true, true, D, false>(g, a, inl, &fz);
}
template <int D, int WM, int NT>
__global__ __launch_bounds__(FW_BLOCK) __attribute__((amdgpu_waves_per_eu(FW_FIFO_WAVES))) void fw_k_update_fifo_far(FwGlobals g, FwFifoArgs a, FwInlineOps inl, FwFuseArgs fz,
                                                                                                                    FwFarArgs far) {
    static_assert(D > FW_FUSE_MAX && D <= FW_FUSE_FAR, "the far tier's depths");
    fw_update_fifo_body<false, WM, NT, 0, FW_ROUNDS, false, true, true, D, true>(g, a, inl, &fz, &far);
}
#ifndef FW_NEST_WAVES
#define FW_NEST_WAVES 4
#endif
template <int NT, int TR>
__global__ __launch_bounds__(FW_BLOCK) __attribute__((amdgpu_waves_per_eu(FW_NEST_WAVES))) void fw_k_update_fifo_nest(FwGlobals g, FwFifoArgs a, FwInlineOps inl) {
    fw_update_fifo_body<false, -1, NT, false, TR, true>(g, a, inl);
}


__device__ __forceinline__ void fw_store_destroyed_vals(char *dbuf, size_t d, const FwType &T, float4 q0, float4 q1, float4 q2,
                                                        float4 q3, float age_new, const float bc[4], const float em[4], float sc) {
    float *rec = reinterpret_cast<float *>(dbuf) + d * 26;
    q2 = fw_record_rotation(T, q2);
    rec[0] = q0.x, rec[1] = q0.y, rec[2] = q0.z;
    rec[3] = q1.x, rec[4] = q1.y, rec[5] = q1.z;
    rec[6] = q2.x, rec[7] = q2.y, rec[8] = q2.z, rec[9] = q2.w;
    rec[10] = q3.x, rec[11] = q3.y, rec[12] = q3.z;
    rec[13] = q1.w, rec[14] = sc, rec[15] = age_new, rec[16] = q3.w;
    rec[17] = bc[0], rec[18] = bc[1], rec[19] = bc[2], rec[20] = bc[3];
    rec[21] = em[0], rec[22] = em[1], rec[23] = em[2], rec[24] = em[3];
    reinterpret_cast<int32_t *>(rec)[25] = T.pbr;
}

template <bool NT = false>
__device__ __forceinline__ void fw_range_inst_out(char *inst, uint32_t inst_cap, const float4 *s_inst_wave, const float4 *rec,
                                                  uint32_t lane, unsigned long long m, uint32_t idx, bool reversed) {
    if (inst == nullptr || m == 0ull) return;
    const uint32_t cnt = (uint32_t)__popcll(m);
    const uint32_t i_lo_lane = __builtin_amdgcn_readlane(idx, __ffsll((long long)m) - 1);
    const uint32_t i_hi_lane = __builtin_amdgcn_readlane(idx, 63 - __clzll((long long)m));
    const uint32_t lowest = reversed ? i_hi_lane : i_lo_lane, highest = reversed ? i_lo_lane : i_hi_lane;
    if (highest - lowest + 1u == cnt) {
        fw_inst_flush<NT>(inst, inst_cap, s_inst_wave, lane, m, lowest);
    } else {
        __builtin_amdgcn_fence(__ATOMIC_RELEASE, "wavefront");
        __builtin_amdgcn_wave_barrier();
        __builtin_amdgcn_fence(__ATOMIC_ACQUIRE, "wavefront");
        if (((m >> lane) & 1ull) && idx < inst_cap)
            for (uint32_t k = 0; k < 4; k++) fw_st4(inst + (size_t)idx * 64u, k, rec[k]);
        __builtin_amdgcn_fence(__ATOMIC_RELEASE, "wavefront");
        __builtin_amdgcn_wave_barrier();
    }
}

#ifndef FW_RANGE_YR
#define FW_RANGE_YR 4
#endif
#ifndef FW_RANGE_PF_ALL
#define FW_RANGE_PF_ALL 1
#endif
#ifndef FW_RINGS_TEMPLATES_ONLY
uint32_t fw_range_young_tile(void) { return FW_RANGE_YR * FW_BLOCK; }
#endif

template <bool ALLNOSPIN, bool INST, int NT, int COLL = 0, int TR = FW_ROUNDS, int YRP = FW_RANGE_YR>
#ifndef FW_RANGE_SPIN_WAVES
#define FW_RANGE_SPIN_WAVES 4
#endif
__global__ __launch_bounds__(FW_BLOCK) __attribute__((amdgpu_waves_per_eu((!ALLNOSPIN && !INST && !COLL && TR == FW_ROUNDS) ? FW_RANGE_SPIN_WAVES : 1)))
void fw_k_update_range(FwGlobals g, FwRangeArgs a) {
    constexpr int BLK = FW_BLOCK;
    constexpr int NW = BLK / 64;
    constexpr int R = TR;
    constexpr int LBW = 4;
    constexpr uint32_t TILE = (uint32_t)(BLK * TR);
    __shared__ __attribute__((aligned(16))) float s_keys[FW_KEYS_MAX];
    __shared__ __attribute__((aligned(16))) float4 s_inst[INST ? NW * 256 : 1];
    __shared__ uint32_t s_cnt[R][NW];
    __shared__ uint32_t s_lb[2 * LBW * NW];
    const uint32_t tid = threadIdx.x, lane = tid & 63u, wave = tid >> 6;
    const FwRangeDesc &D = a.desc[blockIdx.x];
    const uint32_t seg = D.seg, role = D.role_k >> 30;
    uint32_t k = D.role_k & 0x3FFFFFFFu;
    uint32_t ticket = 0u;
    if (FW_TICKETS && role == FW_RANGE_OLD && threadIdx.x == 0u) ticket = atomicAdd(&g.range_ticket[seg], 1u);
#ifdef FW_RANGE_SLEEP
    __builtin_amdgcn_s_sleep(FW_RANGE_SLEEP);
#endif
#ifdef FW_RANGE_STAMP
    struct Stamp {
        unsigned long long *p;
        __device__ ~Stamp() {
            if (p && threadIdx.x == 0) p[3] = __builtin_amdgcn_s_memrealtime();
        }
    } stamp{FW_DBG(a.dbg, 8u) && a.ts ? a.ts + (size_t)blockIdx.x * 8u : nullptr};
    if (stamp.p && tid == 0) stamp.p[0] = __builtin_amdgcn_s_memrealtime(), stamp.p[4] = D.role_k, stamp.p[5] = seg;
#define FW_STAMP(i, dep) do { if (stamp.p && tid == 0) stamp.p[i] = __builtin_amdgcn_s_memrealtime() + ((unsigned long long)(dep) & 0ull); } while (0)
#else
#define FW_STAMP(i, dep) do { } while (0)
#endif
    const bool nospin = ALLNOSPIN || (D.type_idx & FW_TYPE_IDX_NOSPIN) != 0u;
    const uint32_t m2 = nospin ? 0u : 0xFFFFFFFFu;
    const uint32_t keys_off = D.keys_off, keys_len = D.keys_len;
    const float key0 = tid < keys_len ? g.keys[keys_off + tid] : 0.0f;
    const FwRangeRec &Rc = a.recs[seg];
    const uint32_t b = Rc.b, n_spawn_h = Rc.n_spawn, rflags = Rc.flags;
    uint32_t y_exist = Rc.y_exist;
    const FwSeg *Sp = &g.segs[seg];
    const uint32_t C = Sp->capacity;
    char *buf = Sp->buf[0];
    const uint32_t sidx = a.parity * g.max_seg + seg, oidx = (a.parity ^ 1u) * g.max_seg + seg;
    uint32_t y_full = 0xFFFFFFFFu, n_old_dev = 0u;
    if (rflags & (FW_RREC_MAT | FW_RREC_DEV)) {
        const uint32_t c0 = g.count[sidx], c1 = g.spawned[sidx] + g.appended[sidx];
        n_old_dev = g.rold[sidx] + Rc.grad;
        y_full = c0 - min(c0, n_old_dev);
        y_exist = y_full + c1;
    }
    if (blockIdx.x == 0 && tid == 0) {
        if (a.live_next) *a.live_next = 0ull;
        if (a.done_tag) *a.done_tag = a.done_value;
    }
    const char *p0 = buf + FW_OFF_Q0(C), *p1 = buf + FW_OFF_Q1(C), *p2 = buf + FW_OFF_Q2(C), *p3 = buf + FW_OFF_Q3(C);
    const size_t cp = FW_CP(C);
    const char *pl = nospin ? buf + FW_OFF_L(C, Sp->n_lplanes) : p3 + 3 * cp;
    char *inst = INST ? Sp->inst : nullptr;
    const uint32_t inst_cap = INST ? Sp->inst_cap : 0u;
    float4 *s_inst_wave = s_inst + (INST ? wave * 256u : 0u);

    if (role == FW_RANGE_YOUNG) {
        constexpr int YR = TR == FW_ROUNDS ? YRP : TR;
        constexpr uint32_t YT = YR * BLK;
        const uint32_t ring_tiles = C / YT;
        const uint32_t need = min(ring_tiles, (b % YT + y_exist + YT - 1u) / YT);
        if (k >= need) return;
        const uint32_t cnt_y = (INST && inst != nullptr && !(rflags & (FW_RREC_MAT | FW_RREC_DEV))) ? g.count[sidx] : 0u;
        const uint32_t rec0 = (rflags & (FW_RREC_MAT | FW_RREC_DEV)) ? n_old_dev : (cnt_y > y_exist ? cnt_y - y_exist : 0u);
        uint32_t pt = b / YT + k;
        if (pt >= ring_tiles) pt -= ring_tiles;
        const uint32_t sbase = pt * YT;
        FW_STAMP(1, sbase);
        uint32_t yi0 = sbase - b;
        if (sbase < b) yi0 += C;
        uint32_t w_lo = sbase, w_n = YT;
        if (y_exist + YT <= C) {
            if (yi0 < y_exist) w_n = min(YT, y_exist - yi0);
            else w_lo = b, w_n = (b >= sbase && b - sbase < YT) ? min(sbase + YT - b, y_exist) : 0u;
        }
        const fw_rsrc r0 = fw_make_rsrc(p0 + (size_t)w_lo * 16u, w_n * 16u);
        const fw_rsrc r1x = fw_make_rsrc(p1 + (size_t)w_lo * 4u, w_n * 4u), r1y = fw_make_rsrc(p1 + cp + (size_t)w_lo * 4u, w_n * 4u);
        const fw_rsrc r1z = fw_make_rsrc(p1 + 2 * cp + (size_t)w_lo * 4u, w_n * 4u);
        const fw_rsrc r1w = fw_make_rsrc(p1 + 3 * cp + (size_t)w_lo * 4u, INST ? w_n * 4u : 0u);
        const bool need_lf = INST || k == 0u || !(D.type_idx & FW_TYPE_IDX_NOLIFE);
        const fw_rsrc rl = fw_make_rsrc(pl + (size_t)w_lo * 4u, need_lf ? w_n * 4u : 0u);
        auto ldq1 = [&](uint32_t ir) -> float4 {
            const uint32_t i4 = ir / 4u;
            float w = 0.0f;
            if constexpr (INST) w = fw_ldb1<NT == 2>(r1w, i4);
            return make_float4(fw_ldb1<NT == 2>(r1x, i4), fw_ldb1<NT == 2>(r1y, i4), fw_ldb1<NT == 2>(r1z, i4), w);
        };
        constexpr int WMODE = INST ? FW_W_MEM : FW_W_MEM_LAZY;
        const int wd0 = (int)(sbase - w_lo) + (int)tid;
        auto woff = [&](int r) -> uint32_t {
// ... 477 lines not shown
```

bevy_firework_amd/csrc/fw_kernels.h:

```cpp
#pragma once
#include <hip/hip_runtime.h>

#include "fw_device.h"
#include "fw_collide.h"
#include "fw_refit.h"
#include "fw_mesh_bounds.h"
#include "fw_fuse2.h"

#ifdef FW_AB
#define FW_DBG(x, bit) (((x) & (bit)) != 0u)
#else
#define FW_DBG(x, bit) (false)
#endif

#define FW_STAT_SLOTS 32
struct FwGlobals {
    FwSeg *segs;
    FwType *types;
    FwTypeColl *type_coll;
    float *keys;
    FwEmit *emits;
    uint32_t *count;
    uint32_t *spawned;
    uint32_t *appended;
// ... 7 lines not shown
    float *tile_box;
    uint32_t *err;
    unsigned long long *err_host;
    unsigned long long *stats;
    unsigned long long *dbg_ts;
    unsigned long long *emit_serial;
    unsigned long long *nest_status;
    unsigned long long *nest_ticket;
    uint32_t *range_ticket;
    uint32_t *nest_start;
#ifndef FW_TICKETS
#define FW_TICKETS 0
#endif
    const FwCollider *colliders;
    uint32_t n_colliders;
    const FwMeshInst *mesh_inst;
    uint32_t n_mesh_inst;
};

struct FwUpdateArgs {
    const uint32_t *seg_tile_first;
    const uint4 *tile_desc;
    uint32_t n_seg;
    uint32_t total_tiles;
    uint32_t parity;
    uint32_t epoch;
    float dt;
    uint32_t spin_limit;
    uint32_t any_inst;
    unsigned long long *done_tag;
    unsigned long long done_value;
    uint32_t new_static;
    unsigned long long *host_counts;
    const FwOp *ops;
    const uint4 *seg_op_first;
    uint32_t n_ops;
    uint32_t dbg;
    uint32_t vt_rounds;
    uint32_t resident_slots;
    uint32_t seg0_type;
    uint32_t use_stream;
    uint32_t seg0_keys_off, seg0_keys_len;
    const char *seg0_ib;
    char *seg0_ob, *seg0_destroyed, *seg0_inst;
    uint32_t seg0_capacity, seg0_n_lplanes, seg0_inst_cap;
    const uint2 *tile_keys;
    unsigned long long *live_out, *live_next;
    const unsigned long long *fc_in;
    unsigned long long *fc_out;
    unsigned long long *fc_zero;
    const uint4 *fce_in;
    uint4 *fce_out;
    uint32_t force_colors;
    uint32_t boxes;
    uint32_t fc_sums;
    uint32_t fc_s2, fc_tag;
    float fc_theta;
    uint4 *fct_out;
    float2 *fcl_out;
};
#define FW_TF_K 256u
struct FwResolveArgs {
    uint4 *fce;
    const uint4 *fct;
    const float2 *fcl;
    const uint4 *tile_desc;
    uint32_t total_tiles, parity, epoch;
    float dt;
};

#define FW_INLINE_OPS 8
struct FwInlineOps {
    FwOp ops[FW_INLINE_OPS];
};

struct FwFifoSeg {
    char *buf;
    char *destroyed, *inst;
    uint32_t inst_cap, capacity, seg, type_idx;
    uint32_t keys_off, keys_len;
    float life;
    uint32_t head;
    uint32_t n_in;
    uint32_t n_spawn;
    uint32_t dead;
    uint32_t op0, op1;
    uint32_t tile0;
    uint32_t tile_first, n_tiles;
    uint32_t spawn_a, n_vt_a, n_vt_b;
    uint32_t mat;
    uint32_t n_lplanes;
    uint32_t nest;
    unsigned long long *report;
};
#define FW_FIFO_PER_LAUNCH 8
struct FwFifoNest {
    uint32_t parent, child;
    uint32_t emit, emit_slot;
    uint32_t status_first;
    uint32_t n_ptiles;
    uint32_t parent_lplane;
    uint32_t tag;
    uint32_t ticket_base;
    float n_count, n_start, n_end;
    float speed, scale;
    uint32_t spin_limit, pad;
};
#define FW_FIFO_NEST_MAX 4
#define FW_FIFO_NEST_CHILD 0x80000000u
#define FW_LDS_OPS 4u
#define FW_FIFO_COLL_TILE FW_BLOCK
struct FwFifoArgs {
    FwFifoSeg s[FW_FIFO_PER_LAUNCH];
    uint32_t n_segs, parity, epoch, dbg;
    float dt;
    uint32_t any_inst;
    uint32_t any_coll;
    uint32_t small_tiles;
    int32_t write_mask;
    unsigned long long *done_tag;
    unsigned long long done_value;
    unsigned long long *host_counts;
    unsigned long long *live_out, *live_next;
    uint32_t n_nest;
    uint32_t q0pl;
    FwFifoNest nest[FW_FIFO_NEST_MAX];
    uint32_t spinless;
    uint32_t fused;
    uint32_t fuse_pad[31];
};
#define FW_FIFO_WHOLE 0
#define FW_FIFO_NEWBORN 1
static_assert((sizeof(FwGlobals) + sizeof(FwFifoArgs)) % 64 == 0, "FwInlineOps starts on a 64-byte line of the kernel arguments");
static_assert(sizeof(FwFifoArgs) == 1440, "the size every form of the FIFO kernel was measured with (profiles/r22/fuse2_ab.txt)");
struct FwFuseArgs {
    float dt_pre[FW_FUSE_MAX - 1];
    uint32_t pad;
    uint32_t spawn_end[FW_FIFO_PER_LAUNCH][FW_FUSE_MAX - 1];
    uint32_t dead[FW_FIFO_PER_LAUNCH][FW_FUSE_MAX - 1];
    float move[FW_FIFO_PER_LAUNCH][4];
};
static_assert(sizeof(FwFuseArgs) == 32 + 2 * FW_FIFO_PER_LAUNCH * (FW_FUSE_MAX - 1) * 4 + FW_FIFO_PER_LAUNCH * 16,
              "dt_pre and a pad word, two tables of FW_FUSE_MAX - 1 words per ring, four words per ring");
static_assert(sizeof(FwGlobals) + sizeof(FwFifoArgs) + sizeof(FwInlineOps) + sizeof(FwFuseArgs) <= 4096, "the fused kernels' arguments fit the 4096-byte kernel-argument limit");
#define FW_FAR_FIRST (FW_FUSE_MAX - 1)
struct FwFarArgs {
    float dt[FW_FUSE_FAR - FW_FUSE_MAX];
    uint32_t spawn_end[FW_FIFO_PER_LAUNCH][FW_FUSE_FAR - FW_FUSE_MAX];
    uint32_t dead[FW_FIFO_PER_LAUNCH][FW_FUSE_FAR - FW_FUSE_MAX];
};
static_assert(sizeof(FwFarArgs) == (FW_FUSE_FAR - FW_FUSE_MAX) * 4 * (1 + 2 * FW_FIFO_PER_LAUNCH), "one dt and, per ring, two boundaries per far frame");
static_assert(sizeof(FwGlobals) + sizeof(FwFifoArgs) + sizeof(FwInlineOps) + sizeof(FwFuseArgs) + sizeof(FwFarArgs) <= 4096,
              "the far kernels' arguments fit the 4096-byte kernel-argument limit");

struct alignas(16) FwRangeRec {
    uint32_t b;
    uint32_t y_exist;
    uint32_t n_spawn;
    uint32_t op0, op_n;
    uint32_t grad;
    uint32_t flags;
    uint32_t ticket_base;
    unsigned long long *report;
    unsigned long long pad2;
};
#define FW_RREC_MAT 1u
#define FW_RREC_DEV 2u
#define FW_RANGE_OLD 0u
#define FW_RANGE_NEW 1u
#define FW_RANGE_YOUNG 2u
struct alignas(16) FwRangeDesc {
    uint32_t seg;
    uint32_t role_k;
    uint32_t old_first;
    uint32_t type_idx;
    uint32_t keys_off, keys_len;
    uint32_t n_old;
    uint32_t pad;
};
struct FwRangeArgs {
    const FwRangeDesc *desc;
    const FwRangeRec *recs;
    const FwOp *ops;
    unsigned long long *status;
    uint32_t total_tiles, parity, epoch, spin_limit, dbg;
    float dt;
    uint32_t any_inst;
    uint32_t any_coll;
    uint32_t small_tiles;
    uint32_t young_rounds;
    unsigned long long *done_tag;
    unsigned long long done_value;
    unsigned long long *host_counts;
    unsigned long long *live_out, *live_next;
    unsigned long long *ts;
};
#define FW_RANGE_MAX_CAPACITY 0x10000000u

struct FwSmallArgs {
    const uint32_t *list;
    uint32_t n, n_narrow, parity, epoch;
    uint32_t any_inst;
    uint32_t any_coll;
    float dt;
    const uint4 *seg_op_first;
    const FwOp *ops;
    uint32_t force_colors, dbg;
    unsigned long long *done_tag;
    unsigned long long done_value;
    unsigned long long *host_counts;
    unsigned long long *live_out, *live_next;
};
hipError_t fw_launch_update_small(hipStream_t s, const FwGlobals &g, const FwSmallArgs &a, hipEvent_t ev_start = nullptr,
                                  hipEvent_t ev_stop = nullptr);

enum { FW_SPAWN_NONE = 0, FW_SPAWN_INLINE = 1, FW_SPAWN_TABLE = 2 };

enum { FW_MODE_FUSED = 0, FW_MODE_SPLIT = 1, FW_MODE_SPLIT_COLL = 2 };

hipError_t fw_launch_spawn(hipStream_t s, const FwGlobals &g, const FwOp *d_ops, const FwOp *h_ops, uint32_t n_ops,
                           uint32_t total_blocks, uint32_t parity);
hipError_t fw_launch_fc_resolve(hipStream_t s, const FwGlobals &g, const FwResolveArgs &a);
hipError_t fw_launch_update(hipStream_t s, const FwGlobals &g, const FwUpdateArgs &a, const FwInlineOps *inl,
                            int spawn_form, int mode, hipEvent_t ev_start = nullptr, hipEvent_t ev_stop = nullptr);
hipError_t fw_launch_update_fifo2(hipStream_t s, const FwGlobals &g, const FwFifoArgs &a, const FwInlineOps &inl, const FwFuseArgs &fz,
                                  uint32_t total_tiles, int nt, hipEvent_t e0, hipEvent_t e1);
hipError_t fw_launch_update_fifo2_eager(hipStream_t s, const FwGlobals &g, const FwFifoArgs &a, const FwInlineOps &inl, const FwFuseArgs &fz,
                                        uint32_t total_tiles, int nt, hipEvent_t e0, hipEvent_t e1);
hipError_t fw_launch_update_fifo_far(hipStream_t s, const FwGlobals &g, const FwFifoArgs &a, const FwInlineOps &inl, const FwFuseArgs &fz,
                                     const FwFarArgs &far, uint32_t total_tiles, int nt, hipEvent_t e0, hipEvent_t e1);
hipError_t fw_launch_update_fifo(hipStream_t s, const FwGlobals &g, const FwFifoArgs &a, const FwInlineOps &inl,
                                 uint32_t total_tiles, int nt, hipEvent_t ev_start = nullptr, hipEvent_t ev_stop = nullptr, const FwFuseArgs *fz = nullptr);
uint32_t fw_range_young_tile(void);
hipError_t fw_launch_update_range(hipStream_t s, const FwGlobals &g, const FwRangeArgs &a, bool all_nospin, int nt,
                                  hipEvent_t ev_start = nullptr, hipEvent_t ev_stop = nullptr);
hipError_t fw_launch_nested(hipStream_t s, const FwGlobals &g, const FwNestOp *d_ops, const FwNestOp *h_ops, uint32_t n_ops,
                            uint32_t total_tiles, uint32_t parity, uint32_t tag, uint32_t spin_limit, uint32_t dbg = 0);
struct FwSegView {
    char *buf;
    uint32_t capacity;
    uint32_t head;
    const uint32_t *d_rold;
    uint32_t cpl;
    uint32_t nospin;
    float4 rot;
    uint32_t life_plane;
    float life_const;
    const FwType *derived;
    const float *keys;
};
hipError_t fw_launch_gather(hipStream_t s, const FwSegView &v, uint32_t n, int32_t pbr, void *d_out);
hipError_t fw_launch_rederive(hipStream_t s, const FwSegView &v);
hipError_t fw_launch_fifo_ages(hipStream_t s, char *buf, uint32_t capacity, uint32_t head, uint32_t live, const void *d_table, uint32_t n);
hipError_t fw_launch_fifo_spin(hipStream_t s, char *buf, uint32_t capacity, uint32_t head, uint32_t live, const FwType *type, uint32_t axis,
                               const void *d_table, uint32_t n, uint32_t log_n);
hipError_t fw_launch_fill_plane1(hipStream_t s, char *buf0, char *buf1, size_t plane_off, uint32_t capacity, float v);
hipError_t fw_launch_restore_q3(hipStream_t s, char *buf0, char *buf1, uint32_t capacity, uint32_t life_plane, float life_const, uint32_t cpl);
hipError_t fw_launch_fill_rotation(hipStream_t s, char *buf0, char *buf1, uint32_t capacity, const float rot[4], uint32_t cpl);
hipError_t fw_launch_scatter(hipStream_t s, char *buf, uint32_t capacity, uint32_t n, uint32_t n_lplanes,
                             const void *d_in);
hipError_t fw_launch_fill_colors(hipStream_t s, char *buf0, char *buf1, uint32_t capacity, const float bc[4], const float em[4]);
hipError_t fw_launch_pack_instances(hipStream_t s, const FwSegView &v, const uint32_t *d_count, uint32_t n_upper, void *d_out);
struct FwSortView;
hipError_t fw_launch_depth_keys(hipStream_t s, const FwSegView &v, const uint32_t *d_count, uint32_t n_upper, const FwSortView &sv, uint32_t *d_key,
                                uint32_t *d_idx);
hipError_t fw_launch_sort_pairs(hipStream_t s, const uint32_t *d_count, uint32_t n_upper, uint32_t *scratch, uint32_t *d_idx_out);
hipError_t fw_launch_pack_instances_sorted(hipStream_t s, const FwSegView &v, const uint32_t *d_count, uint32_t n_upper, const uint32_t *d_order,
                                           void *d_out);
hipError_t fw_launch_aabb(hipStream_t s, const FwGlobals &g, const uint32_t *seg_ids, const FwSegView *views, uint32_t n_segs,
                          uint32_t parity, float *d_part, float *h_out8);
hipError_t fw_launch_aabb_from_tiles(hipStream_t s, const FwGlobals &g, const uint32_t *seg_ids, uint32_t n_segs,
                                     uint32_t parity, uint32_t epoch, const uint32_t *d_seg_tile_first, float *h_out8);
struct FwBoxEntry {
    FwSegView v;
    const uint32_t *d_count;
    uint32_t bound;
    uint32_t chunk0;
};
struct FwBoxPlace;
hipError_t fw_launch_boxes(hipStream_t s, const FwBoxEntry *d_tab, uint32_t n_entries, const FwBoxPlace *d_places, uint32_t n_places,
                           uint32_t total_chunks, float *d_part, void *out_records, uint32_t *launches);
hipError_t fw_launch_volumes(hipStream_t s, const FwBoxEntry *d_tab, uint32_t n_entries, const FwBoxPlace *d_places, uint32_t n_places, uint32_t total_chunks,
                             const FwCollider *d_volumes, uint32_t n_volumes, uint32_t *d_part, void *out_counts, uint32_t *launches);
hipError_t fw_launch_total(hipStream_t s, const uint32_t *counts, uint32_t n_seg, unsigned long long *d_out);
hipError_t fw_launch_copy_probe(hipStream_t s, const void *src, void *dst, size_t bytes);
#define FW_REFIT_TAIL 4096u
hipError_t fw_launch_mesh_refit(hipStream_t s, const FwRefit &R, const uint32_t *d_level_off, const uint32_t *h_level_off,
                                uint32_t n_levels);
#define FW_BOUNDS_BLOCK 256
#define FW_BOUNDS_MAX_GRID 256u
struct FwMeshSeed {
    float lo[3], hi[3], pad;
};
uint32_t fw_mesh_bounds_partials(uint32_t n_vertices);
hipError_t fw_launch_mesh_bounds(hipStream_t s, const float *d_xyz, const uint8_t *d_referenced, uint32_t n_vertices, FwVtxAcc *d_partials,
                                 FwMeshRecord *d_rec, FwMeshReport *h_report, const FwMeshSeed *seed);
hipError_t fw_launch_mesh_spheres(hipStream_t s, FwMeshInst *d_inst, uint32_t n_inst, const float4 *nodes, const FwMeshRecord *d_rec,
                                  bool after_update);
hipError_t fw_launch_cast_rays(hipStream_t s, const FwGlobals &g, const void *d_rays, uint64_t n, void *d_hits);
hipError_t fw_launch_project_points(hipStream_t s, const FwGlobals &g, const void *d_points, uint64_t n, void *d_out);
struct FwPathSettings;
hipError_t fw_launch_trace_paths(hipStream_t s, const FwGlobals &g, const FwPathSettings &settings, const void *d_paths, uint64_t n, void *d_out,
                                 void *d_samples);
```

bevy_firework_amd/csrc/fw_withheld.h:

```cpp
#pragma once
#include <string.h>
#include "fw_kernels.h"

struct FwFifoLaunch {
    FwFifoArgs fa;
    FwInlineOps fio;
    FwFuseArgs fz;
    FwFarArgs far;
    uint32_t tiles, n_ops;
    int nt;
    uint32_t depth;
    bool held;
    uint64_t frame[FW_FUSE_FAR];
    uint64_t spin_from[FW_FIFO_PER_LAUNCH];
};

struct FwOffered {
    const FwFifoLaunch *first, *second;
    bool withheld;
};

inline bool fw_op_continues(const FwOp &last, const FwOp &b) {
    return b.seg == last.seg && b.emit == last.emit && b.serial_base == last.serial_base + last.n && b.rel_base == last.rel_base + last.n &&
           memcmp(b.origin_pos, last.origin_pos, sizeof b.origin_pos) == 0 && memcmp(b.origin_rot, last.origin_rot, sizeof b.origin_rot) == 0 &&
           memcmp(b.parent_vel, last.parent_vel, sizeof b.parent_vel) == 0 && memcmp(&b.speed, &last.speed, 4) == 0 && memcmp(&b.scale, &last.scale, 4) == 0;
}

class FwWithheld {
public:
    FwOffered offer(FwFifoLaunch &B, bool candidate, uint32_t depth_max, uint64_t frame) {
        FwOffered o{nullptr, nullptr, false};
        B.depth = 1u, B.held = false, B.frame[0] = frame;
        if (on_ && candidate && slot_[at_].depth < depth_max && join(B, depth_max > FW_FUSE_MAX)) {
            if (B.depth >= depth_max) on_ = false, o.second = &B;
            else keep(slot_[at_], B), o.withheld = true;
            return o;
        }
        o.first = take();
        if (!candidate) {
            o.second = &B;
            return o;
        }
        at_ ^= 1u;
        keep(slot_[at_], B);
        for (uint32_t j = 0; j < B.fa.n_segs; j++) grp_[j] = fw_far_begin(FwFifoFrame{B.fa.s[j].head, B.fa.s[j].n_in, B.fa.s[j].n_spawn, B.fa.s[j].dead});
        on_ = true, o.withheld = true;
        return o;
    }
    const FwFifoLaunch *take() {
        if (!on_) return nullptr;
        on_ = false;
        return &slot_[at_];
    }
    void drop() { on_ = false; }
    uint32_t depth() const { return on_ ? slot_[at_].depth : 0u; }

private:
    static void keep(FwFifoLaunch &P, const FwFifoLaunch &B) {
        P = B;
        P.fa.host_counts = nullptr, P.held = true;
    }
    bool join(FwFifoLaunch &B, bool merge) {
        const FwFifoLaunch &P = slot_[at_];
        FwFifoArgs &fa = B.fa;
        const uint32_t d = P.depth;
        if (d < 1u || d >= FW_FUSE_FAR) return false;
        if (P.fa.n_segs != fa.n_segs || P.fa.write_mask != fa.write_mask || P.n_ops > FW_INLINE_OPS || B.n_ops > FW_INLINE_OPS) return false;
        FwFarGroup grp[FW_FIFO_PER_LAUNCH];
        uint32_t merged = 0;
        for (uint32_t j = 0; j < fa.n_segs; j++) {
            const FwFifoSeg &A = P.fa.s[j], &F = fa.s[j];
            if (A.buf != F.buf || A.seg != F.seg || A.capacity != F.capacity || A.type_idx != F.type_idx || A.keys_off != F.keys_off ||
                A.keys_len != F.keys_len || A.life != F.life || A.mat || F.mat || A.destroyed || F.destroyed || A.nest || F.nest)
                return false;
            grp[j] = grp_[j];
            if (!fw_far_push(F.capacity, grp[j], FwFifoFrame{F.head, F.n_in, F.n_spawn, F.dead})) return false;
            if (merge && A.op0 < A.op1 && F.op0 < F.op1) {
                FwOp b = B.fio.ops[F.op0];
                b.rel_base += grp[j].spawn_end[d - 1u];
                merged += fw_op_continues(P.fio.ops[A.op1 - 1u], b) ? 1u : 0u;
            }
        }
        if (P.n_ops + B.n_ops - merged > FW_INLINE_OPS) return false;
        {
            FwFuseArgs fz = d >= 2u ? P.fz : FwFuseArgs{};
            memcpy(fz.move, B.fz.move, sizeof fz.move);
            B.fz = fz;
            B.far = d > FW_FAR_FIRST ? P.far : FwFarArgs{};
        }
        const uint32_t w = d - 1u;
        (w < FW_FAR_FIRST ? B.fz.dt_pre[w] : B.far.dt[w - FW_FAR_FIRST]) = P.fa.dt;
        FwInlineOps ops;
        uint32_t n = 0, t = 0;
        for (uint32_t j = 0; j < fa.n_segs; j++) {
            const FwFifoSeg &A = P.fa.s[j];
            FwFifoSeg &F = fa.s[j];
            const FwFifoFrame &U = grp[j].U;
            const uint32_t o0 = n;
            for (uint32_t x = A.op0; x < A.op1; x++) ops.ops[n++] = P.fio.ops[x];
            for (uint32_t x = F.op0; x < F.op1; x++) {
                FwOp b = B.fio.ops[x];
                b.rel_base += grp[j].spawn_end[w];
                if (merge && x == F.op0 && n > o0 && fw_op_continues(ops.ops[n - 1u], b)) ops.ops[n - 1u].n += b.n;
                else ops.ops[n++] = b;
            }
            const FwFifoLayout L = fw_fifo_layout(F.capacity, FW_TILE, FW_BLOCK, U.head, U.dead, U.n_in, U.n_in, U.n_spawn);
            F.head = U.head, F.n_in = U.n_in, F.n_spawn = U.n_spawn, F.dead = U.dead;
            (w < FW_FAR_FIRST ? B.fz.spawn_end[j][w] : B.far.spawn_end[j][w - FW_FAR_FIRST]) = grp[j].spawn_end[w];
            (w < FW_FAR_FIRST ? B.fz.dead[j][w] : B.far.dead[j][w - FW_FAR_FIRST]) = grp[j].dead[w];
            F.op0 = o0, F.op1 = n;
            F.spawn_a = L.spawn_a, F.n_vt_a = L.n_vt_a, F.n_vt_b = L.n_vt_b, F.tile0 = L.tile0, F.n_tiles = L.n_tiles;
            F.tile_first = t;
            t += F.n_tiles;
            grp_[j] = grp[j];
        }
        for (uint32_t x = 0; x < n; x++) B.fio.ops[x] = ops.ops[x];
        fa.parity = P.fa.parity, fa.fused = d + 1u;
        B.tiles = t, B.n_ops = n;
        B.frame[d] = B.frame[0];
        for (uint32_t f = 0; f < d; f++) B.frame[f] = P.frame[f];
        B.depth = d + 1u, B.held = true;
        return true;
    }

    bool on_ = false;
    uint32_t at_ = 0;
    FwFifoLaunch slot_[2] = {};
    FwFarGroup grp_[FW_FIFO_PER_LAUNCH];
};
```

Measured before the change: 849.8 billion particles/s.

## Add outer fusion tier fusing up to 24 frames per FIFO update launch

Adds a third fusion tier that withholds and fuses up to 24 (default 20) simulation frames into one FIFO update kernel when there are at most four rings and far fusion is already at maximum depth. A new kernel argument block carries per-frame dt and boundaries for frames beyond the far tier. The withheld-launch logic is reworked to fold each frame into the held slot in place rather than copying whole launch structs. The aim is fewer kernel launches and fewer passes over particle memory per frame, at the cost of larger kernel arguments, more template instantiations and longer update latency. It also skips a clock read when host profiling is off.

```diff
diff --git a/bevy_firework_amd/csrc/fw_engine.h b/bevy_firework_amd/csrc/fw_engine.h
--- a/bevy_firework_amd/csrc/fw_engine.h
+++ b/bevy_firework_amd/csrc/fw_engine.h
@@ -641,6 +641,7 @@
     uint32_t fuse2_min = 384u * FW_TILE;
     uint32_t fuse_depth = FW_FUSE_MAX, fuse_deep_min = 768u * FW_TILE, fuse_wide_min = 768u * FW_TILE;
     uint32_t fuse_far_depth = FW_FUSE_FAR_DEFAULT, fuse_far_min = 768u * FW_TILE;
+    uint32_t fuse_outer_depth = FW_FUSE_OUTER_DEFAULT, fuse_outer_min = 768u * FW_TILE;
     FwWithheld withheld;
     uint64_t fused_launches = 0, fuse2_flushed = 0, fuse_frames = 0;
     bool use_axis = true;
diff --git a/bevy_firework_amd/csrc/fw_engine_api.cpp b/bevy_firework_amd/csrc/fw_engine_api.cpp
--- a/bevy_firework_amd/csrc/fw_engine_api.cpp
+++ b/bevy_firework_amd/csrc/fw_engine_api.cpp
@@ -191,6 +191,8 @@
     if (const char *m = getenv("FW_FUSE_WIDE_MIN")) ctx->fuse_wide_min = (uint32_t)strtoul(m, nullptr, 10);
     if (const char *m = getenv("FW_FUSE_FAR_DEPTH")) ctx->fuse_far_depth = (uint32_t)std::min(std::max(atoi(m), (int)FW_FUSE_MAX), (int)FW_FUSE_FAR);
     if (const char *m = getenv("FW_FUSE_FAR_MIN")) ctx->fuse_far_min = (uint32_t)strtoul(m, nullptr, 10);
+    if (const char *m = getenv("FW_FUSE_OUTER_DEPTH")) ctx->fuse_outer_depth = (uint32_t)std::min(std::max(atoi(m), (int)FW_FUSE_FAR), (int)FW_FUSE_OUTER);
+    if (const char *m = getenv("FW_FUSE_OUTER_MIN")) ctx->fuse_outer_min = (uint32_t)strtoul(m, nullptr, 10);
     if (const char *m = getenv("FW_DERIVED")) ctx->use_derived = atoi(m) != 0, ctx->derive_all = atoi(m) >= 2;
     if (const char *m = getenv("FW_NEST_FUSE")) ctx->nest_fuse = atoi(m) != 0;
     if (const char *m = getenv("FW_SMALL")) ctx->use_small = atoi(m) != 0;
diff --git a/bevy_firework_amd/csrc/fw_engine_launch.cpp b/bevy_firework_amd/csrc/fw_engine_launch.cpp
--- a/bevy_firework_amd/csrc/fw_engine_launch.cpp
+++ b/bevy_firework_amd/csrc/fw_engine_launch.cpp
@@ -396,7 +396,9 @@
     if (fused) ctx->fused_launches++, ctx->fuse_frames += L.depth;
     else if (L.held) ctx->fuse2_flushed++;
     count_whole_tiles(ctx, L.fa), count_newborn(ctx, L.fa);
-    if (L.depth > FW_FUSE_MAX)
+    if (L.depth > FW_FUSE_FAR)
+        FW_HIP(ctx, fw_launch_update_fifo_outer(stream, ctx->g, L.fa, L.fio, L.fz, L.far, L.outer, L.tiles, L.nt, e0, e1));
+    else if (L.depth > FW_FUSE_MAX)
         FW_HIP(ctx, fw_launch_update_fifo_far(stream, ctx->g, L.fa, L.fio, L.fz, L.far, L.tiles, L.nt, e0, e1));
     else
         FW_HIP(ctx, fw_launch_update_fifo(stream, ctx->g, L.fa, L.fio, L.tiles, L.nt, e0, e1, fused ? &L.fz : nullptr));
@@ -434,12 +436,18 @@
     bool deep = true;
     bool wide = true;
     bool far = true;
+    bool outer = true;
     uint32_t n_launches = 0;
     bool sent = false;
 
+    FifoAccum() {
+        memset(&L, 0, offsetof(FwFifoLaunch, far));
+        L.tiles = L.n_ops = 0u, L.nt = 0, L.depth = 0u, L.held = false;
+        memset(L.spin_from, 0, sizeof L.spin_from);
+    }
     void restart() {
         const uint32_t n = n_launches;
-        *this = FifoAccum{};
+        *this = FifoAccum();
         n_launches = n;
     }
     struct Words {
@@ -454,6 +462,8 @@
         const bool candidate = fw_fuse2_candidate(ctx->use_fuse2, quiet, n_launches == 0 && fa.n_segs == ctx->census.n_fifo, fa.spinless != 0u, fusable);
         const uint32_t depth_knob = std::max(2u, std::min(ctx->fuse_depth, (uint32_t)FW_FUSE_MAX));
         const bool go_far = deep && wide && far && ctx->fuse_depth == (uint32_t)FW_FUSE_MAX && fa.fuse_pad[FW_FIFO_NEWBORN] != 0u && ctx->fuse_far_depth > (uint32_t)FW_FUSE_MAX;
+        if (go_far && outer && ctx->fuse_far_depth == (uint32_t)FW_FUSE_FAR && fa.n_segs <= (uint32_t)FW_OUTER_RINGS && ctx->fuse_outer_depth > (uint32_t)FW_FUSE_FAR)
+            return Words{candidate, std::min(ctx->fuse_outer_depth, (uint32_t)FW_FUSE_OUTER)};
         if (go_far) return Words{candidate, std::min(ctx->fuse_far_depth, (uint32_t)FW_FUSE_FAR)};
         return Words{candidate, !deep ? 2u : !wide ? std::min(depth_knob, (uint32_t)FW_FUSE_NARROW) : depth_knob};
     }
@@ -549,6 +559,7 @@
     acc.deep &= in.n_in >= ctx->fuse_deep_min;
     acc.wide &= in.n_in >= ctx->fuse_wide_min;
     acc.far &= in.n_in >= ctx->fuse_far_min;
+    acc.outer &= in.n_in >= ctx->fuse_outer_min;
     acc.L.spin_from[fa.n_segs] = R.spin_from_new;
     memcpy(acc.L.fz.move[fa.n_segs], S.fifo_move, sizeof S.fifo_move);
     FwFifoSeg &F = fa.s[fa.n_segs++];
@@ -621,7 +632,7 @@
     ff.small = !fr.ring_stats.fifo_dev && fr.ring_stats.fifo_parts < (uint64_t)ctx->fifo_small_tiles * FW_TILE;
     ff.coll_real = fr.ring_stats.fifo_coll;
     ff.coll = ff.coll_real || ff.small;
-    FifoAccum acc{};
+    FifoAccum acc;
     FwFifoArgs &fa = acc.L.fa;
     uint32_t nest_status_next = 0;
     const uint32_t nest_tag = fr.fuse ? next_nest_seq(ctx) : 0u;
diff --git a/bevy_firework_amd/csrc/fw_engine_step.cpp b/bevy_firework_amd/csrc/fw_engine_step.cpp
--- a/bevy_firework_amd/csrc/fw_engine_step.cpp
+++ b/bevy_firework_amd/csrc/fw_engine_step.cpp
@@ -457,7 +457,7 @@
     if (!ctx) return FW_EINVAL;
     hipSetDevice(ctx->device);
     FwFrame fr;
-    fr.prof_t = std::chrono::steady_clock::now();
+    if (ctx->host_prof) fr.prof_t = std::chrono::steady_clock::now();
     fr.dt = dt;
     fw_status st = begin_frame(ctx, dt);
     if (!st) st = recover_missing_reports(ctx, dt);
diff --git a/bevy_firework_amd/csrc/fw_fuse2.h b/bevy_firework_amd/csrc/fw_fuse2.h
--- a/bevy_firework_amd/csrc/fw_fuse2.h
+++ b/bevy_firework_amd/csrc/fw_fuse2.h
@@ -118,3 +118,24 @@
     G.depth++;
     return true;
 }
+
+#define FW_FUSE_OUTER 24
+#define FW_FUSE_OUTER_DEFAULT 20
+struct FwOuterGroup {
+    FwFifoFrame U;
+    uint32_t depth;
+    uint32_t spawn_end[FW_FUSE_OUTER];
+    uint32_t dead[FW_FUSE_OUTER];
+};
+FW_HD FwOuterGroup fw_outer_begin(const FwFifoFrame &A) {
+    FwOuterGroup G{};
+    G.U = A, G.depth = 1u, G.spawn_end[0] = A.n_spawn, G.dead[0] = A.dead;
+    return G;
+}
+FW_HD bool fw_outer_push(uint32_t capacity, FwOuterGroup &G, const FwFifoFrame &B) {
+    if (G.depth < 1u || G.depth >= FW_FUSE_OUTER || !fw_fuse2_ok(capacity, G.U, B)) return false;
+    G.U = fw_fuse2_frame(G.U, B);
+    G.spawn_end[G.depth] = G.U.n_spawn, G.dead[G.depth] = B.dead;
+    G.depth++;
+    return true;
+}
diff --git a/bevy_firework_amd/csrc/fw_k_rings.hip b/bevy_firework_amd/csrc/fw_k_rings.hip
--- a/bevy_firework_amd/csrc/fw_k_rings.hip
+++ b/bevy_firework_amd/csrc/fw_k_rings.hip
@@ -178,7 +178,7 @@
 #endif
 template <bool INST, int WM, int NT, int COLL, int TR, bool NEST, bool Q0PL = false, bool SPINLESS = false, int FUSE = 0, bool NBFACT = false>
 __device__ __forceinline__ void fw_update_fifo_body(const FwGlobals &g, const FwFifoArgs &a, const FwInlineOps &inl, const FwFuseArgs *fz = nullptr,
-                                                    const FwFarArgs *far = nullptr) {
+                                                    const FwFarArgs *far = nullptr, const FwOuterArgs *outer = nullptr) {
     constexpr int BLK = FW_BLOCK;
     constexpr int NW = BLK / 64;
     constexpr int R = TR;
@@ -217,18 +217,24 @@
     float4 q0c, q1c, q2c, q3c, q0n, q1n, q2n, q3n;
     q0c = q1c = q2c = q3c = q0n = q1n = q2n = q3n = make_float4(0.f, 0.f, 0.f, 0.f);
     static_assert(!SPINLESS || (Q0PL && !INST && TR == FW_ROUNDS), "the spin-less form: streaming launches of rings with Q0 in planes");
-    static_assert(FUSE == 0 || (SPINLESS && FUSE >= 2 && FUSE <= FW_FUSE_FAR), "several frames in one pass: the spin-less forms only, two to FW_FUSE_FAR");
+    static_assert(FUSE == 0 || (SPINLESS && FUSE >= 2 && FUSE <= FW_FUSE_OUTER), "several frames in one pass: the spin-less forms only, two to FW_FUSE_OUTER");
     auto dt_w = [&](int f) -> float {
+        if constexpr (FUSE > FW_FUSE_FAR)
+            if (f >= FW_OUTER_FIRST) return outer->dt[f - FW_OUTER_FIRST];
         if constexpr (FUSE > FW_FUSE_MAX)
             if (f >= FW_FAR_FIRST) return far->dt[f - FW_FAR_FIRST];
         return fz->dt_pre[f];
     };
     auto spawn_end_w = [&](uint32_t jj, int f) -> uint32_t {
+        if constexpr (FUSE > FW_FUSE_FAR)
+            if (f >= FW_OUTER_FIRST) return outer->spawn_end[jj][f - FW_OUTER_FIRST];
         if constexpr (FUSE > FW_FUSE_MAX)
             if (f >= FW_FAR_FIRST) return far->spawn_end[jj][f - FW_FAR_FIRST];
         return fz->spawn_end[jj][f];
     };
     auto dead_w = [&](uint32_t jj, int f) -> uint32_t {
+        if constexpr (FUSE > FW_FUSE_FAR)
+            if (f >= FW_OUTER_FIRST) return outer->dead[jj][f - FW_OUTER_FIRST];
         if constexpr (FUSE > FW_FUSE_MAX)
             if (f >= FW_FAR_FIRST) return far->dead[jj][f - FW_FAR_FIRST];
         return fz->dead[jj][f];
@@ -587,6 +593,12 @@
     static_assert(D > FW_FUSE_MAX && D <= FW_FUSE_FAR, "the far tier's depths");
     fw_update_fifo_body<false, WM, NT, 0, FW_ROUNDS, false, true, true, D, true>(g, a, inl, &fz, &far);
 }
+template <int D, int WM, int NT>
+__global__ __launch_bounds__(FW_BLOCK) __attribute__((amdgpu_waves_per_eu(FW_FIFO_WAVES))) void fw_k_update_fifo_outer(FwGlobals g, FwFifoArgs a, FwInlineOps inl, FwFuseArgs fz,
+                                                                                                                      FwFarArgs far, FwOuterArgs outer) {
+    static_assert(D > FW_FUSE_FAR && D <= FW_FUSE_OUTER, "the outer tier's depths");
+    fw_update_fifo_body<false, WM, NT, 0, FW_ROUNDS, false, true, true, D, true>(g, a, inl, &fz, &far, &outer);
+}
 #ifndef FW_NEST_WAVES
 #define FW_NEST_WAVES 4
 #endif
diff --git a/bevy_firework_amd/csrc/fw_k_rings_outer.hip b/bevy_firework_amd/csrc/fw_k_rings_outer.hip
--- /dev/null
+++ b/bevy_firework_amd/csrc/fw_k_rings_outer.hip
@@ -0,0 +1,38 @@
+#ifndef FW_RINGS_TEMPLATES_ONLY
+#define FW_RINGS_TEMPLATES_ONLY
+#endif
+#include "fw_k_rings.hip"
+
+template <int D>
+static hipError_t fw_launch_fifo_outer_depth(hipStream_t s, const FwGlobals &g, const FwFifoArgs &a, const FwInlineOps &inl, const FwFuseArgs &fz, const FwFarArgs &far,
+                                             const FwOuterArgs &outer, dim3 grid, dim3 block, int nt, hipEvent_t e0, hipEvent_t e1) {
+    if (nt == 2)
+        FW_LAUNCH_T((fw_k_update_fifo_outer<D, -1, 2>), grid, block, s, e0, e1, g, a, inl, fz, far, outer);
+    else if (nt)
+        FW_LAUNCH_T((fw_k_update_fifo_outer<D, -1, 1>), grid, block, s, e0, e1, g, a, inl, fz, far, outer);
+    else if (a.write_mask == 0)
+        FW_LAUNCH_T((fw_k_update_fifo_outer<D, 0, 0>), grid, block, s, e0, e1, g, a, inl, fz, far, outer);
+    else
+        FW_LAUNCH_T((fw_k_update_fifo_outer<D, -1, 0>), grid, block, s, e0, e1, g, a, inl, fz, far, outer);
+    return hipGetLastError();
+}
+
+hipError_t fw_launch_update_fifo_outer(hipStream_t s, const FwGlobals &g, const FwFifoArgs &a, const FwInlineOps &inl, const FwFuseArgs &fz,
+                                       const FwFarArgs &far, const FwOuterArgs &outer, uint32_t total_tiles, int nt, hipEvent_t e0, hipEvent_t e1) {
+    if (!total_tiles || !a.n_segs || !a.spinless || !a.q0pl || a.any_inst || a.small_tiles || a.any_coll || a.n_nest) return hipErrorInvalidValue;
+    if (a.fuse_pad[FW_FIFO_NEWBORN] == 0u) return hipErrorInvalidValue;
+    if (a.n_segs > FW_OUTER_RINGS) return hipErrorInvalidValue;
+    const dim3 grid(total_tiles), block(FW_BLOCK);
+    static_assert(FW_FUSE_FAR == 16 && FW_FUSE_OUTER == 24, "one instantiation per depth");
+    switch (a.fused) {
+    case 17: return fw_launch_fifo_outer_depth<17>(s, g, a, inl, fz, far, outer, grid, block, nt, e0, e1);
+    case 18: return fw_launch_fifo_outer_depth<18>(s, g, a, inl, fz, far, outer, grid, block, nt, e0, e1);
+    case 19: return fw_launch_fifo_outer_depth<19>(s, g, a, inl, fz, far, outer, grid, block, nt, e0, e1);
+    case 20: return fw_launch_fifo_outer_depth<20>(s, g, a, inl, fz, far, outer, grid, block, nt, e0, e1);
+    case 21: return fw_launch_fifo_outer_depth<21>(s, g, a, inl, fz, far, outer, grid, block, nt, e0, e1);
+    case 22: return fw_launch_fifo_outer_depth<22>(s, g, a, inl, fz, far, outer, grid, block, nt, e0, e1);
+    case 23: return fw_launch_fifo_outer_depth<23>(s, g, a, inl, fz, far, outer, grid, block, nt, e0, e1);
+    case 24: return fw_launch_fifo_outer_depth<24>(s, g, a, inl, fz, far, outer, grid, block, nt, e0, e1);
+    default: return hipErrorInvalidValue;
+    }
+}
diff --git a/bevy_firework_amd/csrc/fw_kernels.h b/bevy_firework_amd/csrc/fw_kernels.h
--- a/bevy_firework_amd/csrc/fw_kernels.h
+++ b/bevy_firework_amd/csrc/fw_kernels.h
@@ -183,6 +183,16 @@
 static_assert(sizeof(FwFarArgs) == (FW_FUSE_FAR - FW_FUSE_MAX) * 4 * (1 + 2 * FW_FIFO_PER_LAUNCH), "one dt and, per ring, two boundaries per far frame");
 static_assert(sizeof(FwGlobals) + sizeof(FwFifoArgs) + sizeof(FwInlineOps) + sizeof(FwFuseArgs) + sizeof(FwFarArgs) <= 4096,
               "the far kernels' arguments fit the 4096-byte kernel-argument limit");
+#define FW_OUTER_FIRST (FW_FUSE_FAR - 1)
+#define FW_OUTER_RINGS 4
+struct FwOuterArgs {
+    float dt[FW_FUSE_OUTER - FW_FUSE_FAR];
+    uint32_t spawn_end[FW_OUTER_RINGS][FW_FUSE_OUTER - FW_FUSE_FAR];
+    uint32_t dead[FW_OUTER_RINGS][FW_FUSE_OUTER - FW_FUSE_FAR];
+};
+static_assert(FW_FUSE_OUTER - FW_FUSE_FAR == 8 && sizeof(FwOuterArgs) == 288, "one dt and, per ring of four, two boundaries per outer frame");
+static_assert(sizeof(FwGlobals) + sizeof(FwFifoArgs) + sizeof(FwInlineOps) + sizeof(FwFuseArgs) + sizeof(FwFarArgs) + sizeof(FwOuterArgs) <= 4096,
+              "the outer kernels' arguments fit the 4096-byte kernel-argument limit");
 
 struct alignas(16) FwRangeRec {
     uint32_t b;
@@ -260,6 +270,8 @@
                                         uint32_t total_tiles, int nt, hipEvent_t e0, hipEvent_t e1);
 hipError_t fw_launch_update_fifo_far(hipStream_t s, const FwGlobals &g, const FwFifoArgs &a, const FwInlineOps &inl, const FwFuseArgs &fz,
                                      const FwFarArgs &far, uint32_t total_tiles, int nt, hipEvent_t e0, hipEvent_t e1);
+hipError_t fw_launch_update_fifo_outer(hipStream_t s, const FwGlobals &g, const FwFifoArgs &a, const FwInlineOps &inl, const FwFuseArgs &fz,
+                                       const FwFarArgs &far, const FwOuterArgs &outer, uint32_t total_tiles, int nt, hipEvent_t e0, hipEvent_t e1);
 hipError_t fw_launch_update_fifo(hipStream_t s, const FwGlobals &g, const FwFifoArgs &a, const FwInlineOps &inl,
                                  uint32_t total_tiles, int nt, hipEvent_t ev_start = nullptr, hipEvent_t ev_stop = nullptr, const FwFuseArgs *fz = nullptr);
 uint32_t fw_range_young_tile(void);
diff --git a/bevy_firework_amd/csrc/fw_withheld.h b/bevy_firework_amd/csrc/fw_withheld.h
--- a/bevy_firework_amd/csrc/fw_withheld.h
+++ b/bevy_firework_amd/csrc/fw_withheld.h
@@ -1,4 +1,5 @@
 #pragma once
+#include <stddef.h>
 #include <string.h>
 #include "fw_kernels.h"
 
@@ -7,11 +8,12 @@
     FwInlineOps fio;
     FwFuseArgs fz;
     FwFarArgs far;
+    FwOuterArgs outer;
     uint32_t tiles, n_ops;
     int nt;
     uint32_t depth;
     bool held;
-    uint64_t frame[FW_FUSE_FAR];
+    uint64_t frame[FW_FUSE_OUTER];
     uint64_t spin_from[FW_FIFO_PER_LAUNCH];
 };
 
@@ -31,9 +33,11 @@
     FwOffered offer(FwFifoLaunch &B, bool candidate, uint32_t depth_max, uint64_t frame) {
         FwOffered o{nullptr, nullptr, false};
         B.depth = 1u, B.held = false, B.frame[0] = frame;
-        if (on_ && candidate && slot_[at_].depth < depth_max && join(B, depth_max > FW_FUSE_MAX)) {
-            if (B.depth >= depth_max) on_ = false, o.second = &B;
-            else keep(slot_[at_], B), o.withheld = true;
+        if (depth_max > FW_FUSE_FAR && B.fa.n_segs > FW_OUTER_RINGS) depth_max = FW_FUSE_FAR;
+        const bool merge = depth_max > FW_FUSE_MAX;
+        if (on_ && candidate && slot_[at_].depth < depth_max && admits(B, merge)) {
+            if (slot_[at_].depth + 1u >= depth_max) close_into(B, merge), on_ = false, o.second = &B;
+            else fold_in(B, merge), o.withheld = true;
             return o;
         }
         o.first = take();
@@ -42,8 +46,8 @@
             return o;
         }
         at_ ^= 1u;
-        keep(slot_[at_], B);
-        for (uint32_t j = 0; j < B.fa.n_segs; j++) grp_[j] = fw_far_begin(FwFifoFrame{B.fa.s[j].head, B.fa.s[j].n_in, B.fa.s[j].n_spawn, B.fa.s[j].dead});
+        begin(slot_[at_], B);
+        for (uint32_t j = 0; j < B.fa.n_segs; j++) grp_[j] = fw_outer_begin(FwFifoFrame{B.fa.s[j].head, B.fa.s[j].n_in, B.fa.s[j].n_spawn, B.fa.s[j].dead});
         on_ = true, o.withheld = true;
         return o;
     }
@@ -56,63 +60,130 @@
     uint32_t depth() const { return on_ ? slot_[at_].depth : 0u; }
 
 private:
-    static void keep(FwFifoLaunch &P, const FwFifoLaunch &B) {
-        P = B;
-        P.fa.host_counts = nullptr, P.held = true;
-    }
-    bool join(FwFifoLaunch &B, bool merge) {
+    static float &dt_of(FwFifoLaunch &L, uint32_t w) {
+        return w < FW_FAR_FIRST ? L.fz.dt_pre[w] : w < FW_OUTER_FIRST ? L.far.dt[w - FW_FAR_FIRST] : L.outer.dt[w - FW_OUTER_FIRST];
+    }
+    static uint32_t &spawn_end_of(FwFifoLaunch &L, uint32_t j, uint32_t w) {
+        return w < FW_FAR_FIRST ? L.fz.spawn_end[j][w] : w < FW_OUTER_FIRST ? L.far.spawn_end[j][w - FW_FAR_FIRST] : L.outer.spawn_end[j][w - FW_OUTER_FIRST];
+    }
+    static uint32_t &dead_of(FwFifoLaunch &L, uint32_t j, uint32_t w) {
+        return w < FW_FAR_FIRST ? L.fz.dead[j][w] : w < FW_OUTER_FIRST ? L.far.dead[j][w - FW_FAR_FIRST] : L.outer.dead[j][w - FW_OUTER_FIRST];
+    }
+    static void begin(FwFifoLaunch &P, const FwFifoLaunch &B) {
+        P.fa = B.fa, P.fio = B.fio;
+        P.fz = FwFuseArgs{}, P.far = FwFarArgs{}, P.outer = FwOuterArgs{};
+        memcpy(P.fz.move, B.fz.move, sizeof P.fz.move);
+        P.tiles = B.tiles, P.n_ops = B.n_ops, P.nt = B.nt, P.depth = 1u, P.held = true;
+        P.frame[0] = B.frame[0];
+        memcpy(P.spin_from, B.spin_from, sizeof P.spin_from);
+        P.fa.host_counts = nullptr;
+    }
+    bool admits(const FwFifoLaunch &B, bool merge) const {
         const FwFifoLaunch &P = slot_[at_];
-        FwFifoArgs &fa = B.fa;
+        const FwFifoArgs &fa = B.fa;
         const uint32_t d = P.depth;
-        if (d < 1u || d >= FW_FUSE_FAR) return false;
+        if (d < 1u || d >= FW_FUSE_OUTER || (d >= FW_FUSE_FAR && fa.n_segs > FW_OUTER_RINGS)) return false;
         if (P.fa.n_segs != fa.n_segs || P.fa.write_mask != fa.write_mask || P.n_ops > FW_INLINE_OPS || B.n_ops > FW_INLINE_OPS) return false;
-        FwFarGroup grp[FW_FIFO_PER_LAUNCH];
         uint32_t merged = 0;
         for (uint32_t j = 0; j < fa.n_segs; j++) {
             const FwFifoSeg &A = P.fa.s[j], &F = fa.s[j];
             if (A.buf != F.buf || A.seg != F.seg || A.capacity != F.capacity || A.type_idx != F.type_idx || A.keys_off != F.keys_off ||
                 A.keys_len != F.keys_len || A.life != F.life || A.mat || F.mat || A.destroyed || F.destroyed || A.nest || F.nest)
                 return false;
-            grp[j] = grp_[j];
-            if (!fw_far_push(F.capacity, grp[j], FwFifoFrame{F.head, F.n_in, F.n_spawn, F.dead})) return false;
+            const FwOuterGroup &G = grp_[j];
+            if (G.depth != d || !fw_fuse2_ok(F.capacity, G.U, FwFifoFrame{F.head, F.n_in, F.n_spawn, F.dead})) return false;
             if (merge && A.op0 < A.op1 && F.op0 < F.op1) {
                 FwOp b = B.fio.ops[F.op0];
-                b.rel_base += grp[j].spawn_end[d - 1u];
+                b.rel_base += G.spawn_end[d - 1u];
                 merged += fw_op_continues(P.fio.ops[A.op1 - 1u], b) ? 1u : 0u;
             }
         }
-        if (P.n_ops + B.n_ops - merged > FW_INLINE_OPS) return false;
+        return P.n_ops + B.n_ops - merged <= FW_INLINE_OPS;
+    }
+    void fold_in(const FwFifoLaunch &B, bool merge) {
+        FwFifoLaunch &P = slot_[at_];
+        const uint32_t d = P.depth, w = d - 1u, n_segs = B.fa.n_segs;
+        const uint32_t parity = P.fa.parity;
+        const float dt_w = P.fa.dt;
+        uint32_t gain[FW_FIFO_PER_LAUNCH], at[FW_FIFO_PER_LAUNCH], n = 0;
+        for (uint32_t j = 0; j < n_segs; j++) {
+            const FwFifoSeg &A = P.fa.s[j], &F = B.fa.s[j];
+            fw_outer_push(F.capacity, grp_[j], FwFifoFrame{F.head, F.n_in, F.n_spawn, F.dead});
+            gain[j] = F.op1 - F.op0, at[j] = n;
+            if (merge && A.op0 < A.op1 && F.op0 < F.op1) {
+                FwOp b = B.fio.ops[F.op0];
+                b.rel_base += grp_[j].spawn_end[w];
+                gain[j] -= fw_op_continues(P.fio.ops[A.op1 - 1u], b) ? 1u : 0u;
+            }
+            n += (A.op1 - A.op0) + gain[j];
+        }
+        for (uint32_t j = n_segs; j-- > 0u;) {
+            const FwFifoSeg &A = P.fa.s[j], &F = B.fa.s[j];
+            const uint32_t old = A.op1 - A.op0;
+            if (at[j] != A.op0 && old) memmove(&P.fio.ops[at[j]], &P.fio.ops[A.op0], old * sizeof(FwOp));
+            uint32_t o = at[j] + old;
+            for (uint32_t x = F.op0; x < F.op1; x++) {
+                FwOp b = B.fio.ops[x];
+                b.rel_base += grp_[j].spawn_end[w];
+                if (x == F.op0 && gain[j] < F.op1 - F.op0) P.fio.ops[o - 1u].n += b.n;
+                else P.fio.ops[o++] = b;
+            }
+        }
+        memcpy(&P.fa.n_segs, &B.fa.n_segs, sizeof(FwFifoArgs) - offsetof(FwFifoArgs, n_segs));
+        P.fa.parity = parity, P.fa.fused = d + 1u, P.fa.host_counts = nullptr;
+        dt_of(P, w) = dt_w;
+        uint32_t t = 0;
+        for (uint32_t j = 0; j < n_segs; j++) {
+            FwFifoSeg &F = P.fa.s[j];
+            const FwFifoFrame &U = grp_[j].U;
+            const uint32_t o0 = at[j], o1 = j + 1u < n_segs ? at[j + 1u] : n;
+            F = B.fa.s[j];
+            const FwFifoLayout L = fw_fifo_layout(F.capacity, FW_TILE, FW_BLOCK, U.head, U.dead, U.n_in, U.n_in, U.n_spawn);
+            F.head = U.head, F.n_in = U.n_in, F.n_spawn = U.n_spawn, F.dead = U.dead;
+            spawn_end_of(P, j, w) = grp_[j].spawn_end[w], dead_of(P, j, w) = grp_[j].dead[w];
+            F.op0 = o0, F.op1 = o1;
+            F.spawn_a = L.spawn_a, F.n_vt_a = L.n_vt_a, F.n_vt_b = L.n_vt_b, F.tile0 = L.tile0, F.n_tiles = L.n_tiles;
+            F.tile_first = t;
+            t += F.n_tiles;
+        }
+        memcpy(P.fz.move, B.fz.move, sizeof P.fz.move);
+        memcpy(P.spin_from, B.spin_from, sizeof P.spin_from);
+        P.tiles = t, P.n_ops = n, P.nt = B.nt;
+        P.frame[d] = B.frame[0];
+        P.depth = d + 1u, P.held = true;
+    }
+    void close_into(FwFifoLaunch &B, bool merge) {
+        const FwFifoLaunch &P = slot_[at_];
+        FwFifoArgs &fa = B.fa;
+        const uint32_t d = P.depth, w = d - 1u;
         {
-            FwFuseArgs fz = d >= 2u ? P.fz : FwFuseArgs{};
+            FwFuseArgs fz = P.fz;
             memcpy(fz.move, B.fz.move, sizeof fz.move);
-            B.fz = fz;
-            B.far = d > FW_FAR_FIRST ? P.far : FwFarArgs{};
-        }
-        const uint32_t w = d - 1u;
-        (w < FW_FAR_FIRST ? B.fz.dt_pre[w] : B.far.dt[w - FW_FAR_FIRST]) = P.fa.dt;
+            B.fz = fz, B.far = P.far, B.outer = P.outer;
+        }
+        dt_of(B, w) = P.fa.dt;
         FwInlineOps ops;
         uint32_t n = 0, t = 0;
         for (uint32_t j = 0; j < fa.n_segs; j++) {
             const FwFifoSeg &A = P.fa.s[j];
             FwFifoSeg &F = fa.s[j];
-            const FwFifoFrame &U = grp[j].U;
+            fw_outer_push(F.capacity, grp_[j], FwFifoFrame{F.head, F.n_in, F.n_spawn, F.dead});
+            const FwFifoFrame &U = grp_[j].U;
             const uint32_t o0 = n;
             for (uint32_t x = A.op0; x < A.op1; x++) ops.ops[n++] = P.fio.ops[x];
             for (uint32_t x = F.op0; x < F.op1; x++) {
                 FwOp b = B.fio.ops[x];
-                b.rel_base += grp[j].spawn_end[w];
+                b.rel_base += grp_[j].spawn_end[w];
                 if (merge && x == F.op0 && n > o0 && fw_op_continues(ops.ops[n - 1u], b)) ops.ops[n - 1u].n += b.n;
                 else ops.ops[n++] = b;
             }
             const FwFifoLayout L = fw_fifo_layout(F.capacity, FW_TILE, FW_BLOCK, U.head, U.dead, U.n_in, U.n_in, U.n_spawn);
             F.head = U.head, F.n_in = U.n_in, F.n_spawn = U.n_spawn, F.dead = U.dead;
-            (w < FW_FAR_FIRST ? B.fz.spawn_end[j][w] : B.far.spawn_end[j][w - FW_FAR_FIRST]) = grp[j].spawn_end[w];
-            (w < FW_FAR_FIRST ? B.fz.dead[j][w] : B.far.dead[j][w - FW_FAR_FIRST]) = grp[j].dead[w];
+            spawn_end_of(B, j, w) = grp_[j].spawn_end[w], dead_of(B, j, w) = grp_[j].dead[w];
             F.op0 = o0, F.op1 = n;
             F.spawn_a = L.spawn_a, F.n_vt_a = L.n_vt_a, F.n_vt_b = L.n_vt_b, F.tile0 = L.tile0, F.n_tiles = L.n_tiles;
             F.tile_first = t;
             t += F.n_tiles;
-            grp_[j] = grp[j];
         }
         for (uint32_t x = 0; x < n; x++) B.fio.ops[x] = ops.ops[x];
         fa.parity = P.fa.parity, fa.fused = d + 1u;
@@ -120,11 +191,10 @@
         B.frame[d] = B.frame[0];
         for (uint32_t f = 0; f < d; f++) B.frame[f] = P.frame[f];
         B.depth = d + 1u, B.held = true;
-        return true;
     }
 
     bool on_ = false;
     uint32_t at_ = 0;
     FwFifoLaunch slot_[2] = {};
-    FwFarGroup grp_[FW_FIFO_PER_LAUNCH];
+    FwOuterGroup grp_[FW_FIFO_PER_LAUNCH];
 };
```

Measured after the change: 664.6 billion particles/s. 21.8% lower.
